# biiiipy/JaxMARL-HFT

Measured on AMD Instinct MI355X. Metric: env steps/sec (whole node), 2-agent MARL, 10-level LOB, NUM_ENVS=4096, higher is better.
Workload: dtype int32

## Files before the change

### jaxmarl-hft_amd/csrc/hftlob.hip

```cpp
#include <hip/hip_runtime.h>
#include <stdint.h>
#include <string.h>
#include <stdio.h>
#include <mutex>
#include <type_traits>
#include <limits.h>

#include "../../include/hftlob.h"
#include "hftlob_internal.h"
#define HFTLOB_BAKED_QUAL static
#include "baked_cfgs.inc"

typedef int32_t i32;
typedef uint32_t u32;
typedef uint8_t u8;
#define DEV __device__ __forceinline__

DEV int lane_id() { return __lane_id(); }
DEV i32 rdl(i32 v, int l) { return __builtin_amdgcn_readlane(v, l); }
DEV i32 wrl(i32 old, i32 val, int l) { return __lane_id() == l ? val : old; }
DEV i32 uni(i32 v) { return __builtin_amdgcn_readfirstlane(v); }
DEV float unif(float v) { return __int_as_float(__builtin_amdgcn_readfirstlane(__float_as_int(v))); }
DEV i32 wadd(i32 a, i32 b) { return (i32)((u32)a + (u32)b); }
DEV i32 wsub(i32 a, i32 b) { return (i32)((u32)a - (u32)b); }
DEV i32 wmul(i32 a, i32 b) { return (i32)((u32)a * (u32)b); }
DEV i32 iabs_(i32 a) { return a < 0 ? wsub(0, a) : a; }
DEV i32 isign(i32 a) { return (a > 0) - (a < 0); }
DEV i32 imax_(i32 a, i32 b) { return a > b ? a : b; }
DEV i32 imin_(i32 a, i32 b) { return a < b ? a : b; }
DEV float i2f(i32 a) { return (float)a; }
DEV i32 f2i(float f) { return (i32)f; }
DEV float bitf(i32 w) { return __int_as_float(w); }
DEV i32 fbit(float f) { return __float_as_int(f); }

DEV i32 ifloordiv(i32 a, i32 b) {
    i32 q = a / b;
    if ((a % b != 0) && ((a < 0) != (b < 0))) q -= 1;
    return q;
}
DEV i32 tick_floordiv(const hftlob_env_cfg& c, i32 a) {
    const u32 d = (u32)c.tick_size;
    const int sh = 31 + (d > 1u ? 32 - __builtin_clz(d - 1u) : 0);
    const u32 n = a < 0 ? ~(u32)a : (u32)a;
    const u32 q = (u32)(((unsigned long long)n * c.tick_magic) >> sh);
    return a < 0 ? (i32)~q : (i32)q;
}
DEV float fmod_exact(float x, float y) {
    const float ax = fabsf(x), ay = fabsf(y), qf = ax / ay;
    if (!(qf < 8388608.0f) | !(ay > 0.0f) | !(ay < INFINITY)) return fmodf(x, y);
    float r = fmaf(-truncf(qf), ay, ax);
    r = r < 0.0f ? r + ay : r;
    return copysignf(r, x);
}
DEV float ffloordiv(float x, float y) {
    float mod = fmod_exact(x, y);
    float div = (x - mod) / y;
    bool ind = (mod != 0.0f) && (((y > 0) - (y < 0)) != ((mod > 0) - (mod < 0)));
    if (ind) div = div - 1.0f;
    return roundf(div);
}

DEV float tick_ffloordiv(const hftlob_env_cfg& c, float x) {
    const float y = (float)c.tick_size, a = fabsf(x);
    const float q = a * __builtin_amdgcn_rcpf(y);
    if (!((a < 16777216.0f) & (q < 524288.0f) & (c.tick_size < (1 << 24)))) return ffloordiv(x, y);
    float k = floorf(q), r = fmaf(-k, y, a);
    if (r < 0.0f) { k -= 1.0f; r += y; }
    else if (r >= y) { k += 1.0f; r -= y; }
    return (x < 0.0f ? -(k + (r != 0.0f ? 1.0f : 0.0f)) : k) + 0.0f;
}

#define DPPX(idv, v, ctrl, rmask) __builtin_amdgcn_update_dpp((idv), (v), (ctrl), (rmask), 0xF, false)
DEV i32 wave_max(i32 v) {
    v = imax_(v, DPPX(INT_MIN, v, 0xB1, 0xF));
    v = imax_(v, DPPX(INT_MIN, v, 0x4E, 0xF));
    v = imax_(v, DPPX(INT_MIN, v, 0x141, 0xF));
    v = imax_(v, DPPX(INT_MIN, v, 0x140, 0xF));
    v = imax_(v, DPPX(INT_MIN, v, 0x142, 0xA));
    v = imax_(v, DPPX(INT_MIN, v, 0x143, 0xC));
    return rdl(v, 63);
}
DEV i32 wave_min(i32 v) {
    v = imin_(v, DPPX(INT_MAX, v, 0xB1, 0xF));
    v = imin_(v, DPPX(INT_MAX, v, 0x4E, 0xF));
    v = imin_(v, DPPX(INT_MAX, v, 0x141, 0xF));
    v = imin_(v, DPPX(INT_MAX, v, 0x140, 0xF));
    v = imin_(v, DPPX(INT_MAX, v, 0x142, 0xA));
    v = imin_(v, DPPX(INT_MAX, v, 0x143, 0xC));
    return rdl(v, 63);
}
DEV i32 wave_sum(i32 v) {
    v = wadd(v, DPPX(0, v, 0xB1, 0xF));
    v = wadd(v, DPPX(0, v, 0x4E, 0xF));
    v = wadd(v, DPPX(0, v, 0x141, 0xF));
    v = wadd(v, DPPX(0, v, 0x140, 0xF));
    v = wadd(v, DPPX(0, v, 0x142, 0xA));
    v = wadd(v, DPPX(0, v, 0x143, 0xC));
    return rdl(v, 63);
}
#define FDPP(v, ctrl, rmask) __int_as_float(DPPX(0, __float_as_int(v), ctrl, rmask))
DEV float wave_fsum(float v) {
    v = v + FDPP(v, 0xB1, 0xF);
    v = v + FDPP(v, 0x4E, 0xF);
    v = v + FDPP(v, 0x141, 0xF);
    v = v + FDPP(v, 0x140, 0xF);
    v = v + FDPP(v, 0x142, 0xA);
    v = v + FDPP(v, 0x143, 0xC);
    return __int_as_float(rdl(__float_as_int(v), 63));
}
DEV unsigned long long ballot(bool p) { return __ballot(p); }
DEV i32 fresh(i32 v) {
    asm volatile("" : "+s"(v));
    return v;
}
DEV i32 sel(bool c, i32 a, i32 b) {
    asm volatile("" : "+v"(a));
    asm volatile("" : "+v"(b));
    return c ? a : b;
}
DEV u32 vkeep(u32 v) {
    asm volatile("" : "+v"(v));
    return v;
}
template <int S> DEV void vkeep_sets(u32 (&v)[S]) {
    if (S == 2) asm volatile("" : "+v"(v[0]), "+v"(v[S - 1]));
    else
#pragma unroll
        for (int r = 0; r < S; ++r) asm volatile("" : "+v"(v[r]));
}
DEV float self(bool c, float a, float b) {
    asm volatile("" : "+v"(a));
    asm volatile("" : "+v"(b));
    return c ? a : b;
}

#ifdef HFTLOB_STAMPS
#define STAMP(var) const unsigned long long var = __builtin_amdgcn_s_memtime()
#ifdef HFTLOB_STAMPS_COARSE
#define SUBSTAMP(var) const unsigned long long var = 0
#define STAMP_ACC(acc, since)
#else
#define SUBSTAMP(var) STAMP(var)
#define STAMP_ACC(acc, since) acc += __builtin_amdgcn_s_memtime() - since
#endif
#else
#define STAMP(var)
#define SUBSTAMP(var)
#define STAMP_ACC(acc, since)
#endif

DEV u32 rotl32(u32 x, int r) { return (x << r) | (x >> (32 - r)); }
DEV void threefry(u32 k0, u32 k1, u32 x0, u32 x1, u32& o0, u32& o1) {
    const u32 k2 = k0 ^ k1 ^ 0x1BD11BDAu;
    x0 += k0;
    x1 += k1;
#define TF_R(r) x0 += x1; x1 = rotl32(x1, r); x1 ^= x0;
#define TF_G1 TF_R(13) TF_R(15) TF_R(26) TF_R(6)
#define TF_G2 TF_R(17) TF_R(29) TF_R(16) TF_R(24)
    TF_G1 x0 += k1; x1 += k2 + 1u;
    TF_G2 x0 += k2; x1 += k0 + 2u;
    TF_G1 x0 += k0; x1 += k1 + 3u;
    TF_G2 x0 += k1; x1 += k2 + 4u;
    TF_G1 x0 += k2; x1 += k0 + 5u;
#undef TF_G1
#undef TF_G2
#undef TF_R
    o0 = x0;
    o1 = x1;
}
struct Key { u32 a, b; };
DEV Key split_key(Key k, int n, int j, bool part) {
    Key o;
    if (part) { threefry(k.a, k.b, 0u, (u32)j, o.a, o.b); return o; }
    u32 y0, y1;
    int m = 2 * j;
    if (m < n) { threefry(k.a, k.b, (u32)m, (u32)(n + m), y0, y1); o.a = y0; }
    else { threefry(k.a, k.b, (u32)(m - n), (u32)m, y0, y1); o.a = y1; }
    m = 2 * j + 1;
    if (m < n) { threefry(k.a, k.b, (u32)m, (u32)(n + m), y0, y1); o.b = y0; }
    else { threefry(k.a, k.b, (u32)(m - n), (u32)m, y0, y1); o.b = y1; }
    return o;
}
DEV u32 random_bits(Key k, int n, int i, bool part) {
    u32 y0, y1;
    if (part) { threefry(k.a, k.b, 0u, (u32)i, y0, y1); return y0 ^ y1; }
    int half = (n + 1) / 2;
    if (i < half) {
        threefry(k.a, k.b, (u32)i, (i + half < n) ? (u32)(i + half) : 0u, y0, y1);
        return y0;
    }
    threefry(k.a, k.b, (u32)(i - half), (i < n) ? (u32)i : 0u, y0, y1);
    return y1;
}
DEV i32 randint_vec(Key k, int n, int j, i32 lo, i32 hi, bool part) {
    Key k1 = split_key(k, 2, 0, part), k2 = split_key(k, 2, 1, part);
    u32 hb = random_bits(k1, n, j, part), lb = random_bits(k2, n, j, part);
    u32 span = (hi <= lo) ? 1u : (u32)hi - (u32)lo;
    u32 mult = 65536u % span;
    mult = (mult * mult) % span;
    u32 off = ((hb % span) * mult + (lb % span)) % span;
    return (i32)((u32)lo + off);
}
DEV i32 action_hi(const hftlob_agent_type_cfg& tc) {
    return tc.kind == HFTLOB_AGENT_EXE && tc.action_space == HFTLOB_EXE_ACT_FIXED_PRICES ? tc.fixed_quant_value
                                                                                         : tc.n_actions;
}
DEV i32 randint(Key k, i32 lo, i32 hi, bool part) { return randint_vec(k, 1, 0, lo, hi, part); }

struct LobCfg {
    i32 maxint, init_id, depth, cancel_mode, t4, check_fill, nO, nT;
};
DEV LobCfg lobcfg(const hftlob_lob_cfg& c) {
    LobCfg o;
    o.maxint = c.maxint; o.init_id = c.init_id; o.depth = c.book_depth; o.cancel_mode = c.cancel_mode;
    o.t4 = c.type_4_interpretation; o.check_fill = c.check_book_fill; o.nO = c.n_orders; o.nT = c.n_trades;
    return o;
}

typedef unsigned long long lmask;
DEV lmask bal(bool p) { return __builtin_amdgcn_ballot_w64(p); }
DEV int ffs64(lmask m) { return m ? (int)__builtin_ctzll(m) : -1; }

extern "C" __device__ i32 __hftlob_writelane(i32 val, i32 lane, i32 old) __asm("llvm.amdgcn.writelane.i32");
DEV i32 wlane(i32 old, i32 val, int l) { return __hftlob_writelane(val, l, old); }

#define ENV_BLOCK 64
DEV void lds_order() { __atomic_signal_fence(__ATOMIC_SEQ_CST); }
DEV void wave_sync() {
    __atomic_signal_fence(__ATOMIC_SEQ_CST);
    __builtin_amdgcn_wave_barrier();
}
DEV void one_wave() {
    if (blockDim.x != ENV_BLOCK) __builtin_trap();
}

enum { FP = 0, FQ, FOID, FTID, FTS, FTNS };

template <int S>
struct Valid {
    lmask m[S];
    bool v[S];
    DEV void init(int n) {
        const int l = lane_id();
#pragma unroll
        for (int r = 0; r < S; ++r) {
            v[r] = (r + 1) * 64 <= n ? true : r * 64 + l < n;
            const int k = n - r * 64;
            m[r] = k >= 64 ? ~0ull : (k <= 0 ? 0ull : ((1ull << k) - 1ull));
        }
    }
};

template <int S> DEV void ldcol(const i32* t, int R, int f, i32 (&o)[S]) {
    const int l = lane_id();
#pragma unroll
    for (int r = 0; r < S; ++r) o[r] = t[f * R + r * 64 + l];
}
DEV i32 ldu(const i32* t, int R, int f, int e) { return uni(t[f * R + e]); }
DEV void ld_msg(const i32* g, int4& x, int4& y) {
    x = reinterpret_cast<const int4*>(g)[0];
    y = reinterpret_cast<const int4*>(g)[1];
}
DEV void stu(i32* t, i32* scr, int R, int f, int e, i32 v) {
    const int l = lane_id();
    *(l == 0 ? t + f * R + e : scr + l) = v;
    lds_order();
}
DEV void st6(i32* t, i32* scr, int R, int e, i32 f0, i32 f1, i32 f2, i32 f3, i32 f4, i32 f5) {
    const int l = lane_id();
    i32 v = f0;
    v = wlane(v, f1, 1); v = wlane(v, f2, 2); v = wlane(v, f3, 3); v = wlane(v, f4, 4); v = wlane(v, f5, 5);
    *(l < 6 ? t + l * R + e : scr + l) = v;
    lds_order();
}
DEV void clr6(i32* t, i32* scr, int R, int e) {
    const int l = lane_id();
    *(l < 6 ? t + l * R + e : scr + l) = -1;
    lds_order();
}
DEV u32 ff1(lmask m) {
    u32 r;
    asm("s_ff1_i32_b64 %0, %1" : "=s"(r) : "s"(m));
    return r;
}
template <int S> DEV int first_slot(const lmask (&m)[S], int fallback) {
    u32 idx = ff1(m[0]);
#pragma unroll
    for (int r = 1; r < S; ++r) idx = min(idx, ff1(m[r]) | (u32)(64 * r));
    return idx == 0xFFFFFFFFu ? fallback : (int)idx;
}
template <int S> DEV int first_true(const bool (&pr)[S], int fallback) {
    lmask m[S];
#pragma unroll
    for (int r = 0; r < S; ++r) m[r] = bal(pr[r]);
    return first_slot(m, fallback);
}
template <int S> DEV i32 sget(const i32 (&a)[S], int e) {
    i32 v = a[0];
#pragma unroll
    for (int k = 1; k < S; ++k) v = (e >> 6) == k ? a[k] : v;
    return rdl(v, e & 63);
}

template <int S>
struct Side {
    i32* t;
    i32* scr;
    i32 best_p, best_q;
    i32 xp;
    i32 pc[S];
    i32 top, top_p, top_ts, top_tns;
    i32 rp, rq;
    lmask rm;
};
template <int S> DEV void side_rec(Side<S>& s, u32 k) {
    s.rp = wlane(s.rp, s.best_p, (int)k);
    s.rq = wlane(s.rq, s.best_q, (int)k);
    asm volatile("s_bitset1_b64 %0, %1" : "+s"(s.rm) : "s"(k));
}

template <int S> DEV void col_set(i32 (&c)[S], int e, i32 v) {
    const int l = lane_id();
#pragma unroll
    for (int r = 0; r < S; ++r) c[r] = (l + 64 * r == e) ? v : c[r];
}

enum : u32 { F_STALE_A = 2, F_STALE_B = 4, F_CLEAN_A = 8, F_CLEAN_B = 16, F_NEG1_A = 32, F_NEG1_B = 64,
             F_PM1_A = 256, F_PM1_B = 512, F_STALE_ANY = 0x40000000u, F_SLOW = 0x80000000u };
constexpr u32 STALE_ANY = F_STALE_ANY;
template <bool ASKS> struct SideBits {
    static constexpr u32 STALE = ASKS ? F_STALE_A : F_STALE_B;
    static constexpr u32 MARK = STALE | STALE_ANY;
    static constexpr u32 CLEAN = ASKS ? F_CLEAN_A : F_CLEAN_B;
    static constexpr u32 NEG1 = ASKS ? F_NEG1_A : F_NEG1_B;
    static constexpr u32 PM1 = ASKS ? F_PM1_A : F_PM1_B;
};
DEV u32 slow_bit(u32 fl) {
    return (fl & (F_CLEAN_A | F_CLEAN_B | F_NEG1_A | F_NEG1_B | F_PM1_A | F_PM1_B)) == (F_CLEAN_A | F_CLEAN_B)
               ? 0u : F_SLOW;
}

template <int S>
struct SideRows {
    int2 x0[S], x1[S], x2[S];
};
template <int S> DEV void fetch_side(SideRows<S>& f, const i32* g, const Valid<S>& V) {
    const int l = lane_id();
#pragma unroll
    for (int r = 0; r < S; ++r) {
        f.x0[r] = f.x1[r] = f.x2[r] = make_int2(-1, -1);
        if (V.v[r]) {
            const int2* row = reinterpret_cast<const int2*>(g + (r * 64 + l) * 6);
            f.x0[r] = row[0]; f.x1[r] = row[1]; f.x2[r] = row[2];
        }
    }
}
template <bool ASKS, int S>
DEV u32 commit_side(Side<S>& s, const SideRows<S>& f, int R, const Valid<S>& V) {
    const int l = lane_id();
    lmask bad = 0, n1 = 0, pm1 = 0;
#pragma unroll
    for (int r = 0; r < S; ++r) {
        const int sl = r * 64 + l;
        const i32 p = f.x0[r].x, q = f.x0[r].y, oid = f.x1[r].x, tid = f.x1[r].y, ts = f.x2[r].x, tns = f.x2[r].y;
        if (V.v[r]) {
            i32* t = s.t + sl;
            t[FP * R] = p; t[FQ * R] = q; t[FOID * R] = oid; t[FTID * R] = tid; t[FTS * R] = ts; t[FTNS * R] = tns;
        }
        s.pc[r] = V.v[r] ? p : -1;
        const u32 np_ = ~(u32)p, nq = ~(u32)q, no = ~(u32)oid, nt = ~(u32)tid, ns = ~(u32)ts, nn = ~(u32)tns;
        const u32 any0 = min(min(min(np_, nq), min(no, nt)), min(ns, nn));
        const u32 all0 = max(max(max(np_, nq), max(no, nt)), max(ns, nn));
        bad |= V.m[r] & bal((q <= 0) & (all0 != 0u));
        n1 |= V.m[r] & bal((p != -1) & (any0 == 0u));
        pm1 |= V.m[r] & bal((p == -1) & (all0 != 0u));
    }
    lds_order();
    s.top = -1;
    return (bad == 0ull ? SideBits<ASKS>::CLEAN : 0u) | (n1 != 0ull ? SideBits<ASKS>::NEG1 : 0u) |
           (pm1 != 0ull ? SideBits<ASKS>::PM1 : 0u);
}
template <int S> DEV void relink_side(Side<S>& s, int R, const Valid<S>& V) {
    i32 p[S];
    ldcol(s.t, R, FP, p);
#pragma unroll
    for (int r = 0; r < S; ++r) s.pc[r] = V.v[r] ? p[r] : -1;
    s.top = -1;
}
template <bool ASKS, int S> DEV u32 load_side(Side<S>& s, const i32* g, int R, const Valid<S>& V) {
    SideRows<S> f;
    fetch_side(f, g, V);
    return commit_side<ASKS>(s, f, R, V);
}
template <int S> DEV void store_side(const Side<S>& s, i32* g, int R, const Valid<S>& V) {
    const int l = lane_id();
#pragma unroll
    for (int r = 0; r < S; ++r) {
        const int sl = r * 64 + l;
        if (V.v[r]) {
            const i32* t = s.t + sl;
            int2* row = reinterpret_cast<int2*>(g + sl * 6);
            row[0] = make_int2(t[FP * R], t[FQ * R]);
            row[1] = make_int2(t[FOID * R], t[FTID * R]);
            row[2] = make_int2(t[FTS * R], t[FTNS * R]);
        }
    }
}
template <int S> DEV void clear_masked(Side<S>& s, int R, const lmask (&m)[S]) {
    const int l = lane_id();
#pragma unroll
    for (int r = 0; r < S; ++r) {
        const bool hit = (m[r] >> l) & 1ull;
        s.pc[r] = hit ? -1 : s.pc[r];
        if (hit) {
#pragma unroll
            for (int f = 0; f < 6; ++f) s.t[f * R + r * 64 + l] = -1;
        }
    }
    lds_order();
    s.top = -1;
}

template <bool ASKS, int S> DEV void rzn(Side<S>& s, u32& fl, int R, const Valid<S>& V) {
    i32 q[S];
    ldcol(s.t, R, FQ, q);
    lmask m[S];
#pragma unroll
    for (int r = 0; r < S; ++r) m[r] = V.m[r] & bal(q[r] <= 0);
    clear_masked(s, R, m);
    fl = fl | SideBits<ASKS>::CLEAN | SideBits<ASKS>::MARK;
    fl = (fl & ~F_SLOW) | slow_bit(fl);
}

template <int S> DEV void best_bid_pq(const i32 (&p)[S], const i32 (&q)[S], const Valid<S>& V, i32& bp, i32& bq) {
    i32 m = INT_MIN;
#pragma unroll
    for (int r = 0; r < S; ++r) m = imax_(m, V.v[r] ? p[r] : INT_MIN);
    const i32 mp = wave_max(m);
    i32 v = 0;
#pragma unroll
    for (int r = 0; r < S; ++r) v = wadd(v, (V.v[r] & (p[r] == mp)) ? q[r] : 0);
    bp = mp;
    bq = wave_sum(v);
}
template <int S>
DEV void best_ask_pq(const i32 (&p)[S], const i32 (&q)[S], const Valid<S>& V, i32 maxint, i32& bp, i32& bq,
                     i32* xp = nullptr) {
    i32 m = INT_MAX;
#pragma unroll
    for (int r = 0; r < S; ++r) m = imin_(m, V.v[r] ? (p[r] == -1 ? maxint : p[r]) : INT_MAX);
    const i32 mn = wave_min(m);
    if (xp) *xp = mn;
    const i32 pa = mn == maxint ? -1 : mn;
    i32 v = 0;
#pragma unroll
    for (int r = 0; r < S; ++r) v = wadd(v, (V.v[r] & (p[r] == pa)) ? q[r] : 0);
    bp = pa;
    bq = wave_sum(v);
}
template <bool ASKS, bool REC, int S>
DEV void rescan(Side<S>& s, u32& fl, int R, const Valid<S>& V, i32 maxint, u32 k) {
    i32 q[S];
    ldcol(s.t, R, FQ, q);
    if (ASKS) best_ask_pq(s.pc, q, V, maxint, s.best_p, s.best_q, &s.xp);
    else best_bid_pq(s.pc, q, V, s.best_p, s.best_q);
    fl &= ~SideBits<ASKS>::STALE;
    if (REC) side_rec(s, k);
}

template <int S>
DEV int top_idx(const i32 (&p)[S], const i32 (&ts)[S], const i32 (&tns)[S], const Valid<S>& V, const LobCfg& c, i32 mp,
                i32& mts_out, i32& mtn_out) {
    i32 t[S], n[S], m = INT_MAX;
#pragma unroll
    for (int r = 0; r < S; ++r) {
        t[r] = (p[r] == mp) ? ts[r] : c.maxint;
        m = imin_(m, V.v[r] ? t[r] : INT_MAX);
    }
    const i32 mts = wave_min(m);
    m = INT_MAX;
#pragma unroll
    for (int r = 0; r < S; ++r) {
        n[r] = (t[r] == mts) ? tns[r] : c.maxint;
        m = imin_(m, V.v[r] ? n[r] : INT_MAX);
    }
    const i32 mtn = wave_min(m);
    mts_out = mts;
    mtn_out = mtn;
    lmask pm[S];
#pragma unroll
    for (int r = 0; r < S; ++r) pm[r] = V.m[r] & bal(n[r] == mtn);
    return first_slot(pm, c.nO - 1);
}

struct Trades {
    i32* t;
    i32* scr;
    int R;
    DEV i32 get(int k, int r) const { return t[k * R + r * 64 + lane_id()]; }
    DEV i32 at(int k, int row) const { return uni(t[k * R + row]); }
};
template <int S> DEV void trades_fill(Trades& T, const Valid<S>& V, i32 v) {
    const int l = lane_id();
#pragma unroll
    for (int r = 0; r < S; ++r)
        if (V.v[r]) {
#pragma unroll
            for (int k = 0; k < 8; ++k) T.t[k * T.R + r * 64 + l] = v;
        }
    lds_order();
}
template <int S> DEV void load_trades(Trades& T, const i32* g, const Valid<S>& V) {
    const int l = lane_id();
#pragma unroll
    for (int r = 0; r < S; ++r) {
        if (V.v[r]) {
            const int o = r * 64 + l, R = T.R;
            const int4* row = reinterpret_cast<const int4*>(g + o * 8);
            const int4 a = row[0], b = row[1];
            T.t[0 * R + o] = a.x; T.t[1 * R + o] = a.y; T.t[2 * R + o] = a.z; T.t[3 * R + o] = a.w;
            T.t[4 * R + o] = b.x; T.t[5 * R + o] = b.y; T.t[6 * R + o] = b.z; T.t[7 * R + o] = b.w;
        }
    }
    lds_order();
}
template <int S> DEV void store_trades(const Trades& T, i32* g, const Valid<S>& V) {
    const int l = lane_id();
#pragma unroll
    for (int r = 0; r < S; ++r) {
        if (V.v[r]) {
            const int o = r * 64 + l, R = T.R;
            int4* row = reinterpret_cast<int4*>(g + o * 8);
            row[0] = make_int4(T.t[0 * R + o], T.t[1 * R + o], T.t[2 * R + o], T.t[3 * R + o]);
            row[1] = make_int4(T.t[4 * R + o], T.t[5 * R + o], T.t[6 * R + o], T.t[7 * R + o]);
        }
    }
}
DEV void trade_put(Trades& T, int e, i32 f0, i32 f1, i32 f2, i32 f3, i32 f4, i32 f5, i32 f6, i32 f7) {
    const int l = lane_id();
    i32 v = f0;
    v = wlane(v, f1, 1); v = wlane(v, f2, 2); v = wlane(v, f3, 3);
    v = wlane(v, f4, 4); v = wlane(v, f5, 5); v = wlane(v, f6, 6); v = wlane(v, f7, 7);
    *(l < 8 ? T.t + l * T.R + e : T.scr + l) = v;
    lds_order();
}

#ifndef HFTLOB_FILT_LOG2
#define HFTLOB_FILT_LOG2 12
#endif
constexpr int FILT_LOG2 = HFTLOB_FILT_LOG2, FILT_WORDS = 1 << (FILT_LOG2 - 5);
constexpr int PAD_FILT = 128, PAD_SCR = PAD_FILT + FILT_WORDS, PAD_WORDS = PAD_SCR + 64;
constexpr int PAD_CARRY = 96;
static_assert(FILT_WORDS >= 64 && FILT_WORDS % 64 == 0 && PAD_WORDS - PAD_SCR == 64, "filter words per lane, 64-word scratch row");
static_assert(PAD_CARRY + 13 <= PAD_FILT, "the rollout's 13 carry words end before the filter words");
__host__ __device__ constexpr int book_words(int nO, int nT) { return 12 * nO + 8 * nT + PAD_WORDS; }
template <int S>
struct Book {
    Side<S> a, b;
    Trades tr;
    Valid<S> vs, vt;
    LobCfg c;
    u32 fl;
    Key ek;
    i32 mi, nmsg;
    i32 ntr;
    bool part;
    i32* filt;
    bool filt_ok;
};

enum { H_ASK = 0, H_BID = 1, H_CNL_ASK = 2, H_CNL_BID = 3, H_NOP = 4, H_KIND = 7, H_DISCARD = 8, H_NEG1 = 16,
       H_PM1 = 32, H_MKT = 64, H_RARE = 128, H_MISS = 256, H_NOID = 512 };
struct Msg {
    i32 h, side, price, qty, oid, tid, t, tns;
    u32 k;
};

template <int S> DEV void top_new(Side<S>& s, int e, i32 np, i32 t, i32 tns, i32 maxint) {
    s.top = ((t != maxint) & (tns != maxint)) ? e : -1;
    s.top_p = np; s.top_ts = t; s.top_tns = tns;
}
template <int S> DEV void top_eq(Side<S>& s, int e, i32 t, i32 tns, i32 maxint) {
    if (fresh(t) > s.top_ts) return;
    asm volatile("");
    if (s.top < 0) return;
    asm volatile("");
    bool earlier = t < s.top_ts;
    if (!earlier) earlier = (tns < s.top_tns) | ((tns == s.top_tns) & (e < s.top));
    if (earlier) {
        s.top = tns != maxint ? e : -1;
        s.top_ts = t; s.top_tns = tns;
    }
}
#define XP_SET(s, v) ((s).xp = (v))
template <bool BID, int S, bool STALE_OK = true, bool NN = false>
DEV void note_add(Side<S>& s, u32& fl, int e, i32 np, i32 nq, i32 t, i32 tns, i32 maxint, u32 k) {
    constexpr u32 STALE = SideBits<!BID>::STALE, MARK = SideBits<!BID>::MARK;
    if (STALE_OK && (fl & STALE)) { s.top = -1; return; }
    const i32 bp = s.best_p;
    if (BID) {
        if (np < bp) {
            if (!NN && bp == -1) fl |= MARK;
        } else if (np > bp) {
            s.best_p = np; s.best_q = nq;
            side_rec(s, k);
            top_new(s, e, np, t, tns, maxint);
        } else if (!NN && bp == -1) {
            fl |= MARK;
        } else {
            s.best_q = wadd(s.best_q, nq);
            side_rec(s, k);
            top_eq(s, e, t, tns, maxint);
        }
    } else if (NN && !STALE_OK) {
        const i32 xp = s.xp;
        if (np > xp) {
        } else if (np < xp) {
            s.best_p = np; s.best_q = nq; XP_SET(s, np); side_rec(s, k); top_new(s, e, np, t, tns, maxint);
        } else if (np == maxint) {
            fl |= MARK;
        } else {
            s.best_q = wadd(s.best_q, nq);
            side_rec(s, k);
            top_eq(s, e, t, tns, maxint);
        }
    } else {
        if (np > bp) {
            if (bp == -1) {
                if (np == maxint) fl |= MARK;
                else { s.best_p = np; s.best_q = nq; XP_SET(s, np); side_rec(s, k); top_new(s, e, np, t, tns, maxint); }
            }
        } else if (np < bp) {
            if (NN || np != -1) { s.best_p = np; s.best_q = nq; XP_SET(s, np); side_rec(s, k); top_new(s, e, np, t, tns, maxint); }
        } else if (!NN && np == -1) {
            fl |= MARK;
        } else if (np != maxint) {
            s.best_q = wadd(s.best_q, nq);
            side_rec(s, k);
            top_eq(s, e, t, tns, maxint);
        }
    }
}
template <bool ASKS, int S> DEV void note_reduce(Side<S>& s, u32& fl, i32 op, i32 dq, u32 k) {
    constexpr u32 STALE = SideBits<ASKS>::STALE, MARK = SideBits<ASKS>::MARK;
    if (fl & STALE) return;
    if (op == s.best_p) {
        if (op == -1) {
            fl |= MARK;
        } else {
            s.best_q = wsub(s.best_q, dq);
            side_rec(s, k);
            if (s.best_q <= 0) fl |= MARK;
        }
    } else {
        asm volatile("");
        u32 f = fl;
        f = fresh(op) == -1 ? f | MARK : f;
        f = fresh(s.best_p) == -1 ? f | MARK : f;
        fl = f;
    }
}

template <int S> DEV void side_put(Side<S>& s, int R, int e, i32 f0, i32 f1, i32 f2, i32 f3, i32 f4, i32 f5) {
    st6(s.t, s.scr, R, e, f0, f1, f2, f3, f4, f5);
    col_set(s.pc, e, f0);
}
template <int S> DEV void side_clr(Side<S>& s, int R, int e) {
    clr6(s.t, s.scr, R, e);
    col_set(s.pc, e, -1);
    s.top = e == s.top ? -1 : s.top;
}
template <int S> DEV void free_slots(const Book<S>& B, const Side<S>& s, lmask (&free)[S]) {
#pragma unroll
    for (int r = 0; r < S; ++r) free[r] = B.vs.m[r] & bal(s.pc[r] == -1);
}

template <int S> DEV bool no_slot(const lmask (&m)[S]) {
    lmask a = 0;
#pragma unroll
    for (int r = 0; r < S; ++r) a |= m[r];
    return a == 0ull;
}

template <bool G, bool ASKS, int S>
DEV i32 match_order(Book<S>& B, Side<S>& s, int top, i32 qtm, const Msg& m, i32 qt, i32 pt, i32 ot, i32 tt) {
    const int R = B.c.nO;
    const i32 newq = imax_(0, wsub(qt, qtm));
    const i32 rem = wsub(qtm, qt);
    int e;
    if (B.ntr >= 0) {
        e = imin_(B.ntr, B.c.nT - 1);
        if (m.t != -1) B.ntr = imin_(B.ntr + 1, B.c.nT);
    } else {
        i32 tr4[S];
        ldcol(B.tr.t, B.tr.R, 4, tr4);
        lmask fm[S];
#pragma unroll
        for (int r = 0; r < S; ++r) fm[r] = B.vt.m[r] & bal(tr4[r] == -1);
        e = first_slot(fm, B.c.nT - 1);
    }
    trade_put(B.tr, e, pt, wmul(wsub(0, m.side), wsub(qt, newq)), ot, m.oid, m.t, m.tns, tt, m.tid);
    if (!G || (B.fl & SideBits<ASKS>::CLEAN)) {
        if (newq <= 0) side_clr(s, R, top);
        else stu(s.t, s.scr, R, FQ, top, newq);
        note_reduce<ASKS>(s, B.fl, pt, wsub(qt, newq), m.k);
    } else {
        stu(s.t, s.scr, R, FQ, top, newq);
        rzn<ASKS>(s, B.fl, R, B.vs);
    }
    return rem;
}

template <bool BID, bool G, int S, bool POS = false>
DEV i32 match_against(Book<S>& B, Side<S>& s, i32 qtm, i32 price, const Msg& m) {
    const int R = B.c.nO;
    if (!POS && fresh(qtm) <= 0) return qtm;
    {
        const i32 bp = s.best_p;
        const i32 mp0 = (!BID && bp == -1) ? B.c.maxint : bp;
        if (__builtin_expect(BID ? mp0 < price : mp0 > price, 1)) return qtm;
    }
    while (qtm > 0) {
        if (B.fl & SideBits<!BID>::STALE) rescan<!BID, true>(s, B.fl, R, B.vs, B.c.maxint, m.k);
        i32 mp = s.best_p;
        if (!BID) {
            if (mp == -1) {
                if (price != B.c.maxint) break;
                mp = B.c.maxint;
            } else if (mp > price) {
                break;
            }
        } else if (mp < price) {
            break;
        }
        int top;
        i32 qt, ot, tt, tp;
        if (s.top >= 0 && s.top_p == mp) {
            top = s.top;
            qt = ldu(s.t, R, FQ, top); ot = ldu(s.t, R, FOID, top); tt = ldu(s.t, R, FTID, top);
            tp = mp;
        } else {
            i32 q[S], o[S], t[S], ts[S], tn[S], mts, mtn;
            ldcol(s.t, R, FTS, ts); ldcol(s.t, R, FTNS, tn);
            ldcol(s.t, R, FQ, q); ldcol(s.t, R, FOID, o); ldcol(s.t, R, FTID, t);
            top = top_idx(s.pc, ts, tn, B.vs, B.c, mp, mts, mtn);
            qt = sget(q, top); ot = sget(o, top); tt = sget(t, top); tp = sget(s.pc, top);
            s.top_p = mp; s.top_ts = mts; s.top_tns = mtn;
            s.top = ((tp == mp) & (mp != -1) & (mp != B.c.maxint) & (mts != B.c.maxint) & (mtn != B.c.maxint))
                        ? top : -1;
        }
        if (fresh(tp) == -1) break;
        asm volatile("");
        if (BID ? tp < price : tp > price) break;
        qtm = match_order<G, !BID>(B, s, top, qtm, m, qt, tp, ot, tt);
    }
    return qtm;
}

template <bool BID, bool G, int S>
DEV void add_order(Book<S>& B, Side<S>& s, const Msg& m, i32 qty, const lmask (&free)[S]) {
    const int R = B.c.nO;
    constexpr u32 CLEAN = SideBits<!BID>::CLEAN, NEG1 = SideBits<!BID>::NEG1, MARK = SideBits<!BID>::MARK,
                  PM1 = SideBits<!BID>::PM1;
    const i32 nq = imax_(0, qty);
    if (!G) {
        const int e = first_slot(free, R - 1);
        const bool was_empty = !no_slot(free);
        if (nq > 0) {
            side_put(s, R, e, m.price, nq, m.oid, m.tid, m.t, m.tns);
            if (m.h & (H_NEG1 | H_PM1)) B.fl = B.fl | (m.h & H_NEG1 ? NEG1 : 0u) | (m.h & H_PM1 ? PM1 : 0u) | F_SLOW;
            if (was_empty) note_add<BID>(s, B.fl, e, m.price, nq, m.t, m.tns, B.c.maxint, m.k);
            else { B.fl |= MARK; s.top = -1; }
        } else if (!was_empty) {
            side_clr(s, R, e);
            B.fl |= MARK;
        }
        return;
    }
    lmask fm[S];
    i32 q[S];
    ldcol(s.t, R, FQ, q);
    if ((B.fl & (CLEAN | NEG1 | PM1)) == CLEAN) {
#pragma unroll
        for (int r = 0; r < S; ++r) fm[r] = free[r];
    } else {
        i32 o[S], t[S], ts[S], tn[S];
        ldcol(s.t, R, FOID, o); ldcol(s.t, R, FTID, t);
        ldcol(s.t, R, FTS, ts); ldcol(s.t, R, FTNS, tn);
#pragma unroll
        for (int r = 0; r < S; ++r)
            fm[r] = B.vs.m[r] & (bal(s.pc[r] == -1) | bal(q[r] == -1) | bal(o[r] == -1) | bal(t[r] == -1) |
                                 bal(ts[r] == -1) | bal(tn[r] == -1));
    }
    const int e = first_slot(fm, R - 1);
    if (!(B.fl & CLEAN)) {
        side_put(s, R, e, m.price, nq, m.oid, m.tid, m.t, m.tns);
        if (m.h & H_PM1) B.fl |= PM1;
        rzn<!BID>(s, B.fl, R, B.vs);
        return;
    }
    const i32 op = sget(s.pc, e), oq = sget(q, e);
    const bool was_empty = (op == -1) & (oq == -1);
    if (nq > 0) {
        side_put(s, R, e, m.price, nq, m.oid, m.tid, m.t, m.tns);
        if (m.h & H_NEG1) B.fl |= NEG1;
        if (m.h & H_PM1) B.fl |= PM1;
        if (was_empty) note_add<BID>(s, B.fl, e, m.price, nq, m.t, m.tns, B.c.maxint, m.k);
        else { B.fl |= MARK; s.top = -1; }
    } else if (!was_empty) {
        side_clr(s, R, e);
        B.fl |= MARK;
    }
}

template <bool BID, int S> DEV void evict_if_full(Book<S>& B, Side<S>& s, lmask (&free)[S]) {
    const int R = B.c.nO;
    lmask neg = 0;
#pragma unroll
    for (int r = 0; r < S; ++r) neg |= B.vs.m[r] & bal(s.pc[r] < 0);
    if (neg != 0ull) return;
    i32 w = BID ? INT_MAX : INT_MIN;
#pragma unroll
    for (int r = 0; r < S; ++r)
        w = BID ? imin_(w, B.vs.v[r] ? s.pc[r] : INT_MAX) : imax_(w, B.vs.v[r] ? s.pc[r] : INT_MIN);
    const i32 worst = BID ? wave_min(w) : wave_max(w);
    lmask m[S];
#pragma unroll
    for (int r = 0; r < S; ++r) m[r] = B.vs.m[r] & bal(s.pc[r] == worst);
    const i32 top = s.top;
    clear_masked(s, R, m);
    s.top = worst != s.top_p ? top : -1;
    if ((worst == s.best_p) | (s.best_p == -1)) B.fl |= SideBits<!BID>::MARK;
#pragma unroll
    for (int r = 0; r < S; ++r) free[r] = m[r];
}
template <bool BID, bool RARE, int S, bool POS = false>
DEV void add_free(Book<S>& B, Side<S>& s, const Msg& m, i32 qty, const lmask (&free)[S]) {
    const int R = B.c.nO;
    if (!POS && qty <= 0) return;
    u32 e;
    if (S == 2) {
        if (free[0] != 0ull) {
            e = ff1(free[0]);
            s.pc[0] = wlane(s.pc[0], m.price, (int)e);
        } else {
            e = ff1(free[S - 1]);
            s.pc[S - 1] = wlane(s.pc[S - 1], m.price, (int)e);
            e |= 64u;
        }
        st6(s.t, s.scr, R, (int)e, m.price, qty, m.oid, m.tid, m.t, m.tns);
    } else {
        e = ff1(free[0]);
#pragma unroll
        for (int r = 1; r < S; ++r) e = min(e, ff1(free[r]) | (u32)(64 * r));
        side_put(s, R, (int)e, m.price, qty, m.oid, m.tid, m.t, m.tns);
    }
    if (RARE && __builtin_expect((m.h & (H_NEG1 | H_PM1)) != 0, 0)) {
        asm volatile("");
        constexpr u32 NEG1 = SideBits<!BID>::NEG1, PM1 = SideBits<!BID>::PM1;
        B.fl = B.fl | (m.h & H_NEG1 ? NEG1 : 0u) | (m.h & H_PM1 ? PM1 : 0u) | F_SLOW;
    }
    note_add<BID, S, false, !RARE>(s, B.fl, (int)e, m.price, qty, m.t, m.tns, B.c.maxint, m.k);
}
template <bool BID, int S> DEV bool add_common(Book<S>& B, Side<S>& s, const Msg& m, const lmask (&free)[S]) {
#ifndef HFTLOB_OLD_ADD_TEST
    if (S == 2) {
        if (__builtin_expect(free[0] != 0ull, 1)) {
            add_free<BID, false, S, true>(B, s, m, m.qty, free);
            return true;
        }
        if (free[S - 1] == 0ull) return false;
        add_free<BID, false, S, true>(B, s, m, m.qty, free);
        return true;
    }
#endif
    if (no_slot(free)) return false;
    add_free<BID, false, S, true>(B, s, m, m.qty, free);
    return true;
}
template <bool G, bool RARE, int S> DEV void bid_lim(Book<S>& B, Msg m) {
    if (!RARE) __builtin_assume(m.qty > 0);
    constexpr bool POS = !RARE && !G;
    if (POS) {
        if (__builtin_expect(B.a.xp > m.price, 1)) {
            lmask free[S];
            free_slots(B, B.b, free);
            if (add_common<true>(B, B.b, m, free)) return;
            if (B.c.check_fill) evict_if_full<true>(B, B.b, free);
            add_order<true, G>(B, B.b, m, m.qty, free);
            return;
        }
    }
    const i32 rem = match_against<false, G, S, POS>(B, B.a, m.qty, m.price, m);
    if (RARE && __builtin_expect((m.h & H_MKT) != 0, 0)) m.price = B.c.maxint;
    lmask free[S];
    free_slots(B, B.b, free);
    if (!no_slot(free)) {
        if (!G) add_free<true, RARE>(B, B.b, m, (RARE && (m.h & H_DISCARD)) ? 0 : rem, free);
        else if (!(m.h & H_DISCARD)) add_order<true, G>(B, B.b, m, rem, free);
        return;
    }
    if (B.c.check_fill) evict_if_full<true>(B, B.b, free);
    if (!(m.h & H_DISCARD)) add_order<true, G>(B, B.b, m, rem, free);
}
template <bool G, bool RARE, int S> DEV void ask_lim(Book<S>& B, Msg m) {
    if (!RARE) __builtin_assume(m.qty > 0);
    if (RARE && __builtin_expect((m.h & H_MKT) != 0, 0)) m.price = 0;
    constexpr bool POS = !RARE && !G;
    if (POS && __builtin_expect(B.b.best_p < m.price, 1)) {
        lmask free[S];
        free_slots(B, B.a, free);
        if (add_common<false>(B, B.a, m, free)) return;
        if (B.c.check_fill) evict_if_full<false>(B, B.a, free);
        add_order<false, G>(B, B.a, m, m.qty, free);
        return;
    }
    const i32 rem = match_against<true, G, S, POS>(B, B.b, m.qty, m.price, m);
    lmask free[S];
    free_slots(B, B.a, free);
    if (!no_slot(free)) {
        if (!G) add_free<false, RARE>(B, B.a, m, (RARE && (m.h & H_DISCARD)) ? 0 : rem, free);
        else if (!(m.h & H_DISCARD)) add_order<false, G>(B, B.a, m, rem, free);
        return;
    }
    if (B.c.check_fill) evict_if_full<false>(B, B.a, free);
    if (!(m.h & H_DISCARD)) add_order<false, G>(B, B.a, m, rem, free);
}
template <int S>
DEV int random_id_match(const Book<S>& B, Key& k, const i32 (&o)[S], const lmask (&pm)[S]) {
    k = split_key(k, 2, 0, B.part);
    lmask w[S];
    int tot = 0;
#pragma unroll
    for (int r = 0; r < S; ++r) {
        w[r] = pm[r] & bal(o[r] != 0);
        tot += __builtin_popcountll(w[r]);
    }
    const u32 bits = random_bits(k, 1, 0, B.part);
    const float u = __uint_as_float((bits >> 9) | 0x3f800000u) - 1.0f;
    const float rr = (float)tot * (1.0f - u);
    i32 chosen = 0;
    if (tot > 0) {
        int K = (int)ceilf(rr);
#pragma unroll
        for (int r = 0; r < S; ++r) {
            const int c = __builtin_popcountll(w[r]);
            if (K > 0 && K <= c) {
                const u32 below = __builtin_amdgcn_mbcnt_hi((u32)(w[r] >> 32), __builtin_amdgcn_mbcnt_lo((u32)w[r], 0u));
                const lmask hit = w[r] & bal(below == (u32)(K - 1));
                chosen = rdl(o[r], (int)ff1(hit));
            }
            K -= c;
        }
    }
    lmask f[S];
#pragma unroll
    for (int r = 0; r < S; ++r) f[r] = B.vs.m[r] & bal(o[r] == chosen);
    return first_slot(f, -1);
}
template <bool G, bool ASKS, bool RC, int S> DEV void cancel(Book<S>& B, Side<S>& s, const Msg& m) {
    if (!G && m.qty == 0) return;
    const int R = B.c.nO;
    int idx;
    i32 op, oq;
    if (!RC && (m.h & H_MISS)) {
        idx = R - 1;
        op = sget(s.pc, R - 1);
#ifndef HFTLOB_NO_MISS_EMPTY
        if (!G && fresh(op) == -1) return;
        asm volatile("");
#endif
        oq = ldu(s.t, R, FQ, R - 1);
    } else {
    i32 o[S], q[S];
    ldcol(s.t, R, FOID, o);
    ldcol(s.t, R, FQ, q);
    lmask fm[S];
    idx = -1;
    if (RC || !(m.h & H_NOID)) {
#pragma unroll
        for (int r = 0; r < S; ++r) fm[r] = B.vs.m[r] & bal(o[r] == m.oid);
        idx = first_slot(fm, -1);
    }
    if (idx < 0) {
        const i32 lo = wsub(B.c.init_id, wmul(B.c.depth, 2));
        const u32 span = (u32)wsub(B.c.init_id, lo);
        u32 d[S];
#pragma unroll
        for (int r = 0; r < S; ++r) d[r] = (u32)wsub(o[r], lo);
        vkeep_sets(d);
#pragma unroll
        for (int r = 0; r < S; ++r) d[r] = s.pc[r] == m.price ? d[r] : 0xFFFFFFFFu;
        vkeep_sets(d);
#pragma unroll
        for (int r = 0; r < S; ++r) d[r] = q[r] >= m.qty ? d[r] : 0xFFFFFFFFu;
        vkeep_sets(d);
#pragma unroll
        for (int r = 0; r < S; ++r) fm[r] = B.vs.m[r] & bal(d[r] <= span);
        if (!RC) {
            idx = first_slot(fm, R - 1);
        } else {
            idx = first_slot(fm, -1);
            if (idx < 0 && B.c.cancel_mode >= 2) {
                Key k = split_key(B.ek, B.nmsg, B.mi, B.part);
#pragma unroll
                for (int r = 0; r < S; ++r) fm[r] = B.vs.m[r] & bal(s.pc[r] == m.price) & bal(q[r] >= m.qty);
                idx = random_id_match(B, k, o, fm);
                if (idx < 0 && B.c.cancel_mode == 3) {
#pragma unroll
                    for (int r = 0; r < S; ++r) fm[r] = B.vs.m[r] & bal(s.pc[r] == m.price);
                    idx = random_id_match(B, k, o, fm);
                }
            }
            if (idx < 0) idx = R - 1;
        }
    }
    op = sget(s.pc, idx);
    oq = sget(q, idx);
    }
    if (!G && fresh(op & oq) == -1) {
        asm volatile("");
        if (m.qty >= -1) return;
#ifndef HFTLOB_NO_MISS_EMPTY
        B.fl |= SideBits<ASKS>::PM1 | F_SLOW;
#endif
    }
    const i32 nq = wsub(oq, m.qty);
    if (!G || (B.fl & SideBits<ASKS>::CLEAN)) {
        if (nq <= 0) side_clr(s, R, idx);
        else stu(s.t, s.scr, R, FQ, idx, nq);
        note_reduce<ASKS>(s, B.fl, op, wsub(oq, nq > 0 ? nq : 0), m.k);
    } else {
        stu(s.t, s.scr, R, FQ, idx, nq);
        rzn<ASKS>(s, B.fl, R, B.vs);
    }
}

DEV void decode_msgs(const LobCfg& c, int4& x, const int4& y) {
    const i32 ty = x.x, sd = ty == 4 ? wsub(0, x.y) : x.y;
    const bool cnl = (ty == 2) | (ty == 3);
    i32 h = H_ASK;
    h = (((ty == 0) & (sd == 0))) ? H_NOP : h;
    h = (((ty == 1) | (ty == 4)) & (sd == 1)) ? H_BID : h;
    h = (cnl & (sd == 1)) ? H_CNL_BID : h;
    h = (cnl & (sd == -1)) ? H_CNL_ASK : h;
    if (((c.t4 == 0) | (c.t4 == 2)) & (ty == 4)) h |= H_DISCARD;
    const i32 p_add = c.t4 == 2 ? (h == H_BID ? c.maxint : 0) : x.w;
    if ((p_add != -1) & ((y.x == -1) | (y.y == -1) | (y.z == -1) | (y.w == -1))) h |= H_NEG1;
    if (p_add == -1) h |= H_PM1;
    if (c.t4 == 2) h |= H_MKT;
    if (h & (H_DISCARD | H_NEG1 | H_PM1 | H_MKT)) h |= H_RARE;
    if ((h <= H_BID) & (x.z <= 0)) h |= H_RARE;
    if (((h & H_KIND) == H_ASK) & (sd != -1)) h |= H_RARE;
    if ((h <= H_BID) & (x.w < 0)) h |= H_RARE;
    x.x = h;
    x.y = sd;
}
template <bool G, bool RC, int S>
DEV void process_msg_(Book<S>& B, u32 k, i32 h, i32 sdv, i32 d2, i32 d3, i32 d4, i32 d5, i32 d6, i32 d7) {
    Msg m;
    m.h = h; m.side = 0; m.price = d3; m.qty = d2; m.oid = d4; m.tid = d5; m.t = d6; m.tns = d7;
    m.k = k;
    const i32 kind = h & H_KIND;
    if (kind == H_CNL_ASK) cancel<G, true, RC>(B, B.a, m);
    else if (kind == H_CNL_BID) cancel<G, false, RC>(B, B.b, m);
    else if (kind == H_BID) {
        if (!G && !(h & H_RARE)) {
            m.side = 1;
            bid_lim<G, false>(B, m);
        } else {
            m.side = rdl(sdv, k);
            bid_lim<G, true>(B, m);
        }
    } else if (kind == H_ASK) {
        if (!G && !(h & H_RARE)) {
            m.side = -1;
            ask_lim<G, false>(B, m);
        } else {
            m.side = rdl(sdv, k);
            ask_lim<G, true>(B, m);
        }
    }
}

DEV i32 ffill(i32 v, i32 carry) {
    const int l = lane_id();
    const lmask m = bal(v != -1) & (~0ull >> (63 - l));
    const int src = m ? 63 - __builtin_clzll(m) : -1;
    const i32 got = __builtin_amdgcn_ds_bpermute(src << 2, v);
    return src < 0 ? carry : got;
}
template <bool REC = true, int S> DEV void refresh_best(Book<S>& B, u32 k = 0) {
    if (B.fl & STALE_ANY) {
        if (B.fl & F_STALE_A) rescan<true, REC>(B.a, B.fl, B.c.nO, B.vs, B.c.maxint, k);
        if (B.fl & F_STALE_B) rescan<false, REC>(B.b, B.fl, B.c.nO, B.vs, B.c.maxint, k);
        B.fl &= ~STALE_ANY;
    }
}

DEV u32 hash_id(i32 v) { return ((u32)v * 0x9E3779B1u) >> (32 - FILT_LOG2); }
DEV u32 hash_px(i32 p, bool ask) { return (((u32)p * 0x85EBCA6Bu) ^ (ask ? 0xC2B2AE35u : 0x27D4EB2Fu)) >> (32 - FILT_LOG2); }
DEV void filt_set(i32* f, u32 h, bool on) {
    __hip_atomic_fetch_or(reinterpret_cast<u32*>(f) + (h >> 5), on ? 1u << (h & 31) : 0u, __ATOMIC_RELAXED,
                          __HIP_MEMORY_SCOPE_WORKGROUP);
}
DEV u32 filt_get(const i32* f, u32 h) { return ((u32)f[h >> 5] >> (h & 31)) & 1u; }
DEV u32 lanes_below(lmask m) { return __builtin_amdgcn_mbcnt_hi((u32)(m >> 32), __builtin_amdgcn_mbcnt_lo((u32)m, 0u)); }
template <int S> DEV int side_room(const Book<S>& B, const Side<S>& s) {
    const int R = B.c.nO, rl = (R - 1) >> 6, ll = (R - 1) & 63;
    int n = 0;
    bool last = false;
#pragma unroll
    for (int r = 0; r < S; ++r) {
        lmask f = B.vs.m[r] & bal(s.pc[r] == -1);
        if (r == rl) {
            last = (f >> ll) & 1ull;
            f &= ~(1ull << ll);
        }
        n += __builtin_popcountll(f);
    }
    if (!last) return -1;
    return ldu(s.t, R, FQ, R - 1) == -1 ? n : -1;
}
template <bool RC, int S> DEV lmask chunk_noops(Book<S>& B, const int4& x, const int4& y, int cnt, i32& hf) {
    const int l = lane_id();
    const i32 kind = x.x & H_KIND, qty = x.z, price = x.w, oid = y.x;
    const bool in = l < cnt;
    const lmask nop = bal(in & (kind == H_NOP));
    hf = 0;
    if ((i32)B.fl < 0) {
        B.filt_ok = false;
        return nop;
    }
    const bool cnl = (kind == H_CNL_ASK) | (kind == H_CNL_BID), add = (kind == H_ASK) | (kind == H_BID);
    const i32 lo = wsub(B.c.init_id, wmul(B.c.depth, 2));
    const u32 span = (u32)wsub(B.c.init_id, lo);
    const bool init_oid = (u32)wsub(oid, lo) <= span;
    const lmask brk = bal(in & ((add & (((x.x & (H_NEG1 | H_PM1)) != 0) | init_oid)) | (cnl & (qty < -1))));
    const lmask before = brk ? (1ull << ff1(brk)) - 1ull : ~0ull;
    const lmask zero = bal(in & cnl & (qty == 0)) & before;
    if (RC || (u32)wsub(-1, lo) <= span) return nop | zero;
    i32* f = B.filt;
    if (!B.filt_ok) {
#pragma unroll
        for (int w = 0; w < FILT_WORDS; w += 64) f[w + l] = 0;
        wave_sync();
        const int R = B.c.nO;
#pragma unroll
        for (int sd = 0; sd < 2; ++sd) {
            const Side<S>& s = sd ? B.b : B.a;
            i32 o[S];
            ldcol(s.t, R, FOID, o);
#pragma unroll
            for (int r = 0; r < S; ++r) {
                filt_set(f, hash_id(o[r]), B.vs.v[r] & (o[r] != -1));
                filt_set(f, hash_px(s.pc[r], sd == 0), B.vs.v[r] & ((u32)wsub(o[r], lo) <= span));
            }
        }
    }
    filt_set(f, hash_id(oid), in & add);
    B.filt_ok = brk == 0ull;
    wave_sync();
    const bool ask = kind == H_CNL_ASK;
    const u32 hid = filt_get(f, hash_id(oid)), hpx = filt_get(f, hash_px(price, ask));
    const bool hit = (hid | hpx) != 0u;
    const int room_a = side_room(B, B.a), room_b = side_room(B, B.b);
    const u32 adds_a = lanes_below(bal(in & (kind == H_ASK))), adds_b = lanes_below(bal(in & (kind == H_BID)));
    const int room = ask ? room_a : room_b;
    const i32 adds = (i32)(ask ? adds_a : adds_b);
    const bool cmiss = in & cnl & (oid != -1) & !hit;
    const bool quiet = cmiss & (qty >= -1) & (room >= 0) & (adds <= room);
#ifndef HFTLOB_NO_MISS
    const bool cnd = in & cnl & (oid != -1) & (hid == 0u) & (((before >> l) & 1ull) != 0ull);
    hf = cnd ? (hpx == 0u ? (i32)H_MISS : (i32)H_NOID) : 0;
#endif
    return nop | zero | (bal(quiet) & before);
}

#ifdef HFTLOB_STAMPS_CHUNK
#define CHUNK_PARAMS , unsigned long long &acc_pre, unsigned long long &acc_loop
#define CHUNK_ARGS , acc_pre, acc_loop
#else
#define CHUNK_PARAMS
#define CHUNK_ARGS
#endif
template <bool RC, int S>
DEV void run_chunk(Book<S>& B, const int4& x, const int4& y, int cnt, int base, i32& rpa, i32& rqa, i32& rpb,
                   i32& rqb CHUNK_PARAMS) {
#ifdef HFTLOB_STAMPS_CHUNK
    const unsigned long long tp0 = __builtin_amdgcn_s_memtime();
#endif
    const lmask live = cnt >= 64 ? ~0ull : (1ull << cnt) - 1ull;
#ifdef HFTLOB_NO_SKIP
    const lmask skip = 0;
    const i32 hx = x.x;
#else
    i32 hf;
    const lmask skip = chunk_noops<RC>(B, x, y, cnt, hf) & live;
    const i32 hx = x.x | hf;
#endif
    lmask todo = live & ~skip;
#ifdef HFTLOB_KO_LOOP
    todo = 0;
#endif
    refresh_best<false>(B);
    const i32 cpa = B.a.best_p, cqa = B.a.best_q, cpb = B.b.best_p, cqb = B.b.best_q;
    B.a.rm = B.b.rm = 0ull;
    B.a.rp = B.a.rq = B.b.rp = B.b.rq = 0;
#ifdef HFTLOB_STAMPS_CHUNK
    const unsigned long long tp1 = __builtin_amdgcn_s_memtime();
    acc_pre += tp1 - tp0;
#endif
    if (todo) {
        u32 k = ff1(todo);
        i32 h = rdl(hx, k), d2 = rdl(x.z, k), d3 = rdl(x.w, k), d4 = rdl(y.x, k),
            d5 = rdl(y.y, k), d6 = rdl(y.z, k), d7 = rdl(y.w, k);
        do {
            asm volatile("s_bitset0_b64 %0, %1" : "+s"(todo) : "s"(k));
            if (RC) B.mi = base + (int)k;
            if ((i32)B.fl >= 0) process_msg_<false, RC>(B, k, h, x.y, d2, d3, d4, d5, d6, d7);
            else process_msg_<true, RC>(B, k, h, x.y, d2, d3, d4, d5, d6, d7);
            refresh_best(B, k);
            const u32 kn = ff1(todo);
            h = rdl(hx, kn); d2 = rdl(x.z, kn); d3 = rdl(x.w, kn);
            d4 = rdl(y.x, kn); d5 = rdl(y.y, kn); d6 = rdl(y.z, kn); d7 = rdl(y.w, kn);
            k = kn;
        } while (todo);
    }
#ifdef HFTLOB_STAMPS_CHUNK
    acc_loop += __builtin_amdgcn_s_memtime() - tp1;
#endif
    {
        const int l = lane_id();
        const lmask below = ~0ull >> (63 - l);
        const lmask ma = B.a.rm & below, mb = B.b.rm & below;
        const int sa = ma ? 63 - __builtin_clzll(ma) : -1, sb = mb ? 63 - __builtin_clzll(mb) : -1;
        const i32 gpa = __builtin_amdgcn_ds_bpermute(sa << 2, B.a.rp), gqa = __builtin_amdgcn_ds_bpermute(sa << 2, B.a.rq);
        const i32 gpb = __builtin_amdgcn_ds_bpermute(sb << 2, B.b.rp), gqb = __builtin_amdgcn_ds_bpermute(sb << 2, B.b.rq);
        rpa = sa < 0 ? cpa : gpa;
        rqa = sa < 0 ? cqa : gqa;
        rpb = sb < 0 ? cpb : gpb;
        rqb = sb < 0 ? cqb : gqb;
    }
}

template <int S> DEV void book_bind(Book<S>& B, i32* lds) {
    B.a.t = lds;
    B.b.t = lds + 6 * B.c.nO;
    B.tr.t = lds + 12 * B.c.nO;
    B.tr.R = B.c.nT;
    B.filt = lds + 12 * B.c.nO + 8 * B.c.nT + PAD_FILT;
    B.filt_ok = false;
    B.a.scr = B.b.scr = B.tr.scr = lds + 12 * B.c.nO + 8 * B.c.nT + PAD_SCR;
    B.vs.init(B.c.nO);
    B.vt.init(B.c.nT);
}

template <int S, bool RC>
__global__ __launch_bounds__(64) void k_book_process(hftlob_lob_cfg cfg, int n_env, int n_msg, const u32* __restrict__ keys,
                                                     const i32* __restrict__ msgs,
                                                     i32* __restrict__ asks, i32* __restrict__ bids,
                                                     i32* __restrict__ trades, i32* __restrict__ best_asks,
                                                     i32* __restrict__ best_bids) {
    one_wave();
    extern __shared__ __attribute__((aligned(16))) i32 lds[];
    const int e = blockIdx.x;
    if (e >= n_env) return;
    const int l = lane_id();
    Book<S> B;
    B.c = lobcfg(cfg);
    book_bind(B, lds);
    const int R = B.c.nO;
    i32* ga = asks + (size_t)e * R * 6;
    i32* gb = bids + (size_t)e * R * 6;
    i32* gt = trades + (size_t)e * B.c.nT * 8;
    B.fl = load_side<true>(B.a, ga, R, B.vs) | load_side<false>(B.b, gb, R, B.vs) | F_STALE_A | F_STALE_B | STALE_ANY;
    B.fl |= slow_bit(B.fl);
    load_trades(B.tr, gt, B.vt);
    {
        lmask fr[S], bad = 0;
#pragma unroll
        for (int r = 0; r < S; ++r) fr[r] = B.vt.m[r] & bal(B.tr.get(4, r) == -1);
        const int first = first_slot(fr, B.c.nT);
        const int l = lane_id();
#pragma unroll
        for (int r = 0; r < S; ++r) bad |= B.vt.m[r] & ~fr[r] & bal(r * 64 + l >= first);
        B.ntr = bad == 0ull ? first : -1;
    }
    if (RC) {
        B.ek = Key{keys[2 * e], keys[2 * e + 1]};
        B.nmsg = n_msg;
        B.part = cfg.prng_partitionable;
    }
    const i32* gm = msgs + (size_t)e * n_msg * 8;
    int4 nx = make_int4(0, 0, 0, 0), ny = nx;
    if (l < n_msg) {
        ld_msg(gm + l * 8, nx, ny);
    }
    for (int base = 0; base < n_msg; base += 64) {
        const int row = base + l;
        int4 x = nx, y = ny;
        nx = make_int4(0, 0, 0, 0);
        ny = nx;
        if (row + 64 < n_msg) {
            ld_msg(gm + (row + 64) * 8, nx, ny);
        }
        decode_msgs(B.c, x, y);
        i32 ap = 0, aq = 0, bp = 0, bq = 0;
        const int cnt = uni(imin_(64, n_msg - base));
#ifdef HFTLOB_STAMPS_CHUNK
        unsigned long long acc_pre = 0, acc_loop = 0;
#endif
        run_chunk<RC>(B, x, y, cnt, base, ap, aq, bp, bq CHUNK_ARGS);
        if (best_asks && row < n_msg) {
            reinterpret_cast<int2*>(best_asks + ((size_t)e * n_msg + row) * 2)[0] = make_int2(ap, aq);
            reinterpret_cast<int2*>(best_bids + ((size_t)e * n_msg + row) * 2)[0] = make_int2(bp, bq);
        }
    }
    store_side(B.a, ga, R, B.vs);
    store_side(B.b, gb, R, B.vs);
    store_trades(B.tr, gt, B.vt);
}

struct EnvCfg {
    const hftlob_env_cfg* c;
};

enum { LD_T0 = 0, LD_T1, LD_WIN, LD_MAXS, LD_START, LD_STEP };
enum { W_T0 = 0, W_T1, W_OIDC, W_MID, W_DT };

DEV int agent_words(const hftlob_agent_type_cfg& t) { return t.kind == HFTLOB_AGENT_MM ? 5 : 13; }

template <int S> DEV i32 side_volume_pq(const i32 (&p)[S], const i32 (&q)[S], const Valid<S>& V) {
    i32 v = 0;
#pragma unroll
    for (int r = 0; r < S; ++r) v = wadd(v, (V.v[r] && p[r] != -1) ? q[r] : 0);
    return wave_sum(v);
}
template <int S> DEV i32 side_volume(const Side<S>& s, int R, const Valid<S>& V) {
    i32 q[S];
    ldcol(s.t, R, FQ, q);
    return side_volume_pq(s.pc, q, V);
}
template <int S> DEV void global_pq(const i32* g, const Valid<S>& V, i32 (&p)[S], i32 (&q)[S]) {
    const int l = lane_id();
#pragma unroll
    for (int r = 0; r < S; ++r) {
        p[r] = q[r] = -1;
        if (V.v[r]) {
            const int2 x = reinterpret_cast<const int2*>(g + (r * 64 + l) * 6)[0];
            p[r] = x.x; q[r] = x.y;
        }
    }
}

struct DivBatch {
    int l;
    float n = 0.0f, d = 1.0f, q = 0.0f;
    DEV void add(int k, float num, float den) {
        n = l == k ? num : n;
        d = l == k ? den : d;
    }
    DEV void run() { q = n / d; }
    DEV float get(int k) const { return unif_lane(q, k); }
    DEV static float unif_lane(float v, int k) { return __int_as_float(__builtin_amdgcn_readlane(__float_as_int(v), k)); }
};
DEV float zsum(float z, int n) { return n >= 64 ? z : z + 0.0f; }
template <int S> DEV float rows_fsum(const float (&x)[S], int n) {
    const int l = lane_id();
    float a = l < n ? x[0] : 0.0f;
#pragma unroll
    for (int r = 1; r < S; ++r) if (r * 64 + l < n) a = a + x[r];
    return wave_fsum(a);
}

struct ObsLane {
    int l;
    float v = 0.0f, off = 0.0f, div = 1.0f;
    DEV void put(int k, float x, float o, float d) {
        const bool me = l == k;
        v = me ? x : v;
        off = me ? o : off;
        div = me ? d : div;
    }
    DEV void put_i(int k, i32 x) { v = l == k ? __int_as_float(x) : v; }
    DEV float fin() const { return (v - off) / div; }
};

struct WorldView {
    i32 best_ask_p, best_bid_p, vol_a, vol_b, step, max_steps;
    float mid;
    i32 t0, t1, it0, it1;
    float dt;
};

#define OBS_F(k, x, o_, d_) o.put((k), (x), nz ? (o_) : 0.0f, nz ? (d_) : 1.0f)
#define OBS_I(k, x, o_, d_) do { if (RAW) o.put_i((k), (x)); else OBS_F((k), i2f(x), (o_), (d_)); } while (0)
template <bool RAW>
DEV void mm_obs(const hftlob_env_cfg& c, const hftlob_agent_type_cfg& tc, const WorldView& w, const i32* st, ObsLane& o,
                bool ftime) {
    const bool nz = !RAW && tc.normalize;
    const i32 spread = iabs_(wsub(w.best_ask_p, w.best_bid_p));
    if (tc.observation_space == HFTLOB_MM_OBS_BASIC) {
        OBS_I(0, st[2], 0.0f, 10.0f);
        OBS_I(1, spread, 0.0f, 1e4f);
        return;
    }
    if (tc.observation_space == HFTLOB_MM_OBS_MESSAGES) return;
    if (ftime) {
        const float tm = i2f(w.t0) + i2f(w.t1) / 1e9f;
        const float trem = (float)c.episode_time - (tm - (i2f(w.it0) + i2f(w.it1) / 1e9f));
        OBS_F(0, w.dt, 0.0f, 10.0f);
        OBS_I(1, st[2], 0.0f, 10.0f);
        OBS_F(2, w.mid, 0.0f, 1e6f);
        OBS_I(3, w.best_ask_p, 0.0f, 1e6f);
        OBS_I(4, w.best_bid_p, 0.0f, 1e6f);
        OBS_I(5, w.vol_a, 0.0f, 1000.0f);
        OBS_I(6, w.vol_b, 0.0f, 1000.0f);
        OBS_I(7, spread, 0.0f, 1e4f);
        OBS_I(8, w.step, 0.0f, 10.0f);
        OBS_F(9, trem, 0.0f, (float)c.episode_time);
        return;
    }
    OBS_I(0, st[2], 0.0f, 10.0f);
    OBS_F(1, w.mid, 0.0f, 1e6f);
    OBS_I(2, w.best_ask_p, 0.0f, 1e6f);
    OBS_I(3, w.best_bid_p, 0.0f, 1e6f);
    OBS_I(4, w.vol_a, 0.0f, 1000.0f);
    OBS_I(5, w.vol_b, 0.0f, 1000.0f);
    OBS_I(6, spread, 0.0f, 1e4f);
    OBS_I(7, w.step, 0.0f, 10.0f);
}
template <bool RAW>
DEV void exe_obs(const hftlob_env_cfg& c, const hftlob_agent_type_cfg& tc, const WorldView& w, const i32* st, ObsLane& o,
                 bool ftime) {
    const bool nz = !RAW && tc.normalize;
    if (tc.observation_space == HFTLOB_EXE_OBS_BASIC) {
        const i32 rq = wsub(st[1], st[2]);
        if (RAW) {
            o.put_i(0, w.best_ask_p);
            o.put_i(1, w.best_bid_p);
        } else {
            o.put(0, i2f(nz ? wsub(w.best_ask_p, 1550000) : w.best_ask_p), 0.0f, nz ? 1e3f : 1.0f);
            o.put(1, i2f(nz ? wsub(w.best_bid_p, 1550000) : w.best_bid_p), 0.0f, nz ? 1e3f : 1.0f);
        }
        OBS_I(2, rq, 0.0f, (float)tc.task_size);
        return;
    }
    if (tc.observation_space == HFTLOB_EXE_OBS_SIMPLEST_CASE) {
        const float ep = (float)c.episode_time;
        const float ptr = (ep - (i2f(wsub(w.t0, w.it0)) + i2f(wsub(w.t1, w.it1)) / 1e9f)) / ep;
        const float prq = i2f(wsub(st[1], st[2])) / i2f(st[1]);
        OBS_F(0, w.mid, 7560000.0f, 1e3f);
        OBS_F(1, prq, 0.5f, 1.0f);
        OBS_F(2, ptr, 0.5f, 1.0f);
        return;
    }
    const i32 sell = st[3];
    const i32 p_aggr = sell ? w.best_bid_p : w.best_ask_p, p_pass = sell ? w.best_ask_p : w.best_bid_p;
    const i32 q_aggr = sell ? w.vol_b : w.vol_a, q_pass = sell ? w.vol_a : w.vol_b;
    const float ip = bitf(st[0]);
    const float ts = (float)tc.task_size;
    const float rr = w.max_steps == 0 ? 0.0f : 1.0f - i2f(w.step) / i2f(w.max_steps);
    const i32 spr = iabs_(wsub(p_aggr, p_pass)), rq = wsub(st[1], st[2]);
    int k = 0;
    if (ftime) {
        OBS_F(0, w.dt, 0.0f, 10.0f);
        k = 1;
    }
    OBS_I(k + 0, st[2], 0.0f, ts);
    OBS_F(k + 1, ip, 0.0f, 1e7f);
    OBS_I(k + 2, sell, 0.0f, 1.0f);
    OBS_I(k + 3, p_aggr, ip, 1e5f);
    OBS_I(k + 4, p_pass, ip, 1e5f);
    OBS_I(k + 5, q_aggr, 0.0f, 1000.0f);
    OBS_I(k + 6, q_pass, 0.0f, 1000.0f);
    OBS_I(k + 7, rq, 0.0f, ts);
    OBS_F(k + 8, rr, 0.0f, 1.0f);
    OBS_I(k + 9, spr, 0.0f, 1e4f);
    OBS_I(k + 10, w.step, 0.0f, 30.0f);
    OBS_I(k + 11, st[1], 0.0f, ts);
    if (ftime) {
        const float tm = i2f(w.t0) + i2f(w.t1) / 1e9f;
        const float trem = (float)c.episode_time - (tm - (i2f(w.it0) + i2f(w.it1) / 1e9f));
        OBS_F(13, tm, 0.0f, 1e5f);
        OBS_F(14, trem, 0.0f, (float)c.episode_time);
    }
}
#undef OBS_I
#undef OBS_F
template <bool RAW>
DEV void write_obs(const hftlob_env_cfg& c, const hftlob_agent_type_cfg& tc, const WorldView& w, const i32* st,
                   void* dst, bool zero, bool ftime) {
    const int l = lane_id();
    ObsLane o{l};
    if (tc.kind == HFTLOB_AGENT_MM) mm_obs<RAW>(c, tc, w, st, o, ftime);
    else exe_obs<RAW>(c, tc, w, st, o, ftime);
    const float v = zero ? 0.0f : (RAW ? o.v : o.fin());
    if (l < c.obs_stride) static_cast<float*>(dst)[l] = v;
}

static_assert(HFTLOB_N_BAKED == 4, "baked_cfg names the table's entries one by one");
template <int BAKED> DEV const hftlob_env_cfg& baked_cfg(const hftlob_env_cfg& rt) {
    static_assert(BAKED >= -1 && BAKED < HFTLOB_N_BAKED, "no such baked config");
    if constexpr (BAKED == 0) return hftlob_baked_cfg_0;
    else if constexpr (BAKED == 1) return hftlob_baked_cfg_1;
    else if constexpr (BAKED == 2) return hftlob_baked_cfg_2;
    else if constexpr (BAKED == 3) return hftlob_baked_cfg_3;
    else return rt;
}
template <int BAKED> constexpr int baked_unroll() { return BAKED >= 0 ? HFTLOB_MAX_AGENTS : 1; }

template <int S, int BAKED = -1>
DEV void env_reset_dev(const hftlob_env_cfg& c_rt, Key key, const i32* __restrict__ init_states, i32* __restrict__ rec,
                       float* __restrict__ obs, const Valid<S>& VS, const Valid<S>& VT, bool ftime) {
    const hftlob_env_cfg& c = baked_cfg<BAKED>(c_rt);
    constexpr int UNR = baked_unroll<BAKED>();
    const bool part = c.prng_partitionable;
    const int nTy = c.n_types, l = lane_id();
    Key wk = split_key(key, nTy + 1, nTy, part);
    i32 idx = c.window_selector == -1 ? randint(wk, 0, c_rt.n_windows, part) : c.window_selector;
    idx = imin_(imax_(idx, 0), c_rt.n_windows - 1);
    const i32* src = init_states + (size_t)idx * c.init_rec_words;
    for (int w = l * 4; w < c.init_rec_words; w += 256) {
        if (w + 3 < c.init_rec_words) {
            *reinterpret_cast<int4*>(rec + w) = *reinterpret_cast<const int4*>(src + w);
        } else {
            for (int k = w; k < c.init_rec_words; ++k) rec[k] = src[k];
        }
    }
    i32 ap[S], aq[S], bp[S], bq[S], ba_p, ba_q, bb_p, bb_q;
    global_pq(src + c.off_asks, VS, ap, aq);
    global_pq(src + c.off_bids, VS, bp, bq);
    best_ask_pq(ap, aq, VS, c.lob.maxint, ba_p, ba_q);
    best_bid_pq(bp, bq, VS, bb_p, bb_q);
    for (int m = l; m < c.n_msgs; m += 64) {
        reinterpret_cast<int2*>(rec + c.off_best_asks)[m] = make_int2(ba_p, ba_q);
        reinterpret_cast<int2*>(rec + c.off_best_bids)[m] = make_int2(bb_p, bb_q);
    }
    const float mid = i2f(wadd(bb_p, ba_p)) / 2.0f;
    const i32 t0 = src[c.off_loaded + LD_T0], t1 = src[c.off_loaded + LD_T1];
    if (l == 0) {
        i32* W = rec + c.off_world;
        W[W_T0] = t0; W[W_T1] = t1; W[W_OIDC] = c.order_id_counter_start; W[W_MID] = fbit(mid); W[W_DT] = fbit(0.0f);
    }
    WorldView wv;
    wv.best_ask_p = ba_p; wv.best_bid_p = bb_p;
    wv.vol_a = side_volume_pq(ap, aq, VS); wv.vol_b = side_volume_pq(bp, bq, VS);
    wv.step = src[c.off_loaded + LD_STEP]; wv.max_steps = src[c.off_loaded + LD_MAXS]; wv.mid = mid;
    wv.t0 = wv.it0 = t0; wv.t1 = wv.it1 = t1; wv.dt = 0.0f;
    int agents_end = c.off_agents;
#pragma unroll UNR
    for (int t = 0; t < nTy; ++t) agents_end += c.types[t].n_agents * agent_words(c.types[t]);
    for (int w = c.off_world + 5 + l; w < c.off_agents; w += 64) rec[w] = 0;
    for (int w = agents_end + l; w < c.rec_words; w += 64) rec[w] = 0;
    i32* st = rec + c.off_agents;
    int ag = 0;
#pragma unroll UNR
    for (int t = 0; t < nTy; ++t) {
        const hftlob_agent_type_cfg& tc = c.types[t];
        i32 sell = tc.task == HFTLOB_TASK_SELL ? 1 : 0;
        if (tc.kind == HFTLOB_AGENT_EXE && tc.task == HFTLOB_TASK_RANDOM)
            sell = randint(split_key(key, nTy + 1, t, part), 0, 2, part);
#pragma unroll UNR
        for (int i = 0; i < tc.n_agents; ++i, ++ag) {
            i32 s[13];
            if (tc.kind == HFTLOB_AGENT_MM) {
                s[0] = 0; s[1] = 0; s[2] = 0; s[3] = fbit(0.0f); s[4] = fbit(0.0f);
            } else {
                s[0] = fbit(mid); s[1] = tc.task_size; s[2] = 0; s[3] = sell; s[4] = fbit(mid / (float)c.tick_size);
                for (int k = 5; k < 13; ++k) s[k] = fbit(0.0f);
            }
            const int nw = agent_words(tc);
            i32 v = 0;
            for (int k = 0; k < 13; ++k) if (l == k) v = s[k];
            if (l < nw) st[l] = v;
            if (obs) write_obs<false>(c, tc, wv, s, obs + (size_t)ag * c.obs_stride, false, ftime);
            st += nw;
        }
    }
}

template <int S>
__global__ __launch_bounds__(64) void k_env_reset(hftlob_env_cfg c, int n_env, const u32* __restrict__ keys,
                                                  const i32* __restrict__ init_states, i32* __restrict__ state,
                                                  float* __restrict__ obs) {
    one_wave();
    const int e = blockIdx.x;
    if (e >= n_env) return;
    Valid<S> VS, VT;
    VS.init(c.lob.n_orders);
    VT.init(c.lob.n_trades);
    Key k{keys[2 * e], keys[2 * e + 1]};
    env_reset_dev<S>(c, k, init_states, state + (size_t)e * c.rec_words,
                     obs ? obs + (size_t)e * c.n_agents * c.obs_stride : nullptr, VS, VT, c.ep_type == 1);
}

struct ActX {
    i32 bid_price, ask_price, bid_dist, ask_dist, bid_quant, ask_quant;
};

DEV void put_row(i32* lds_rows, int row, i32 f0, i32 f1, i32 f2, i32 f3, i32 f4, i32 f5, i32 f6, i32 f7) {
    const int l = lane_id();
    i32 v = f0;
    v = l == 1 ? f1 : v; v = l == 2 ? f2 : v; v = l == 3 ? f3 : v;
    v = l == 4 ? f4 : v; v = l == 5 ? f5 : v; v = l == 6 ? f6 : v; v = l == 7 ? f7 : v;
    if (l < 8) lds_rows[row * 8 + l] = v;
}

template <int S>
struct RegRows {
    int4 x, y;
    i32 meta;
    i32 at[S], aq[S], ao[S], bt[S], bq[S], bo[S];
    DEV void init(const i32* ta, const i32* tb, int R, int C, i32 t, i32 tns) {
        const int l = lane_id();
        const bool cl = l < C;
        x = make_int4(cl ? 2 : 0, 0, 0, 0);
        y = make_int4(0, 0, cl ? t : 0, cl ? tns : 0);
        meta = l | l << 8;
        ldcol(ta, R, FTID, at); ldcol(ta, R, FQ, aq); ldcol(ta, R, FOID, ao);
        ldcol(tb, R, FTID, bt); ldcol(tb, R, FQ, bq); ldcol(tb, R, FOID, bo);
    }
    DEV void put(int row, i32 f0, i32 f1, i32 f2, i32 f3, i32, i32, i32, i32) {
        const bool m = lane_id() == row;
        x.x = m ? f0 : x.x; x.y = m ? f1 : x.y; x.z = m ? f2 : x.z; x.w = m ? f3 : x.w;
    }
    DEV void agent(int arow, int crow, int n, i32 tid, i32 t, i32 tns) {
        const int l = lane_id();
        const bool ia = (u32)(l - arow) < (u32)n, ic = (u32)(l - crow) < (u32)n;
        y.y = ia ? tid : y.y; y.z = ia ? t : y.z; y.w = ia ? tns : y.w;
        const i32 ma = arow | crow << 8 | (n - 1) << 16, mc = crow | arow << 8 | (n - 1) << 16;
        meta = ia ? ma : (ic ? mc : meta);
    }
};
template <int S>
DEV void put_row(RegRows<S>* r, int row, i32 f0, i32 f1, i32 f2, i32 f3, i32 f4, i32 f5, i32 f6, i32 f7) {
    r->put(row, f0, f1, f2, f3, f4, f5, f6, f7);
}
template <class T> struct is_reg_rows { static constexpr bool value = false; };
template <int S> struct is_reg_rows<RegRows<S>*> { static constexpr bool value = true; };
template <bool REG, int S> DEV auto row_sink(RegRows<S>& regs, i32* lds_rows) {
    if constexpr (REG) return &regs;
    else return lds_rows;
}
template <int S>
DEV void cancel_regs(RegRows<S>& sink, const i32 (&tid)[S], const i32 (&q)[S], const i32 (&o)[S], const i32 (&p)[S],
                     const Valid<S>& V, i32 agent, int size, i32 side, int row0) {
    const int l = lane_id();
    sink.x.y = (u32)(l - row0) < (u32)size ? side : sink.x.y;
    int n = 0;
#pragma unroll
    for (int r = 0; r < S; ++r) {
        lmask bm = V.m[r] & bal(tid[r] == agent);
        while (bm && n < size) {
            const int ln = (int)__builtin_ctzll(bm);
            bm &= bm - 1;
            const bool m = l == row0 + n;
            sink.x.z = m ? rdl(q[r], ln) : sink.x.z; sink.x.w = m ? rdl(p[r], ln) : sink.x.w;
            sink.y.x = m ? rdl(o[r], ln) : sink.y.x; sink.y.y = m ? agent : sink.y.y;
            ++n;
        }
    }
}

template <int S>
DEV void cancel_rows(const Side<S>& s, int R, const Valid<S>& V, i32 agent, int size, i32 side, i32 t, i32 tns,
                     i32* lds_rows, int row0) {
    int n = 0;
    i32 tid[S], q[S], o[S];
    const i32 (&p)[S] = s.pc;
    ldcol(s.t, R, FTID, tid);
    ldcol(s.t, R, FQ, q);
    ldcol(s.t, R, FOID, o);
#pragma unroll
    for (int r = 0; r < S; ++r) {
        lmask bm = V.m[r] & bal(tid[r] == agent);
        while (bm && n < size) {
            const int ln = (int)__builtin_ctzll(bm);
            bm &= bm - 1;
            put_row(lds_rows, row0 + n, 2, side, rdl(q[r], ln), rdl(p[r], ln), rdl(o[r], ln), agent, t, tns);
            ++n;
        }
    }
    for (; n < size; ++n) put_row(lds_rows, row0 + n, 2, side, 0, 0, 0, 0, t, tns);
}

template <int n>
DEV void filter_rows(i32* lds_rows, int arow, int crow, i32* scratch) {
    wave_sync();
    const int l = lane_id();
    const bool is_a = l < n, is_c = (l >= 8) & (l < 8 + n);
    const int row = is_a ? arow + l : (is_c ? crow + l - 8 : arow);
    const i32 p = lds_rows[row * 8 + 3], q = lds_rows[row * 8 + 2];
    lmask ma = 0, mc = 0;
#pragma unroll
    for (int k = 0; k < n; ++k) {
        const i32 cpk = rdl(p, 8 + k), apk = rdl(p, k);
        ma |= bal(is_a & (p != 0) & (p == cpk));
        mc |= bal(is_c & (apk != 0) & (p == apk));
    }
    constexpr lmask amask = (1ull << n) - 1, cmask = amask << 8;
    const int na = __builtin_popcountll(ma), nc = __builtin_popcountll(mc);
    const lmask mine = is_a ? ma : mc, all = is_a ? amask : cmask;
    const bool matched = (mine >> l) & 1ull;
    const lmask below = matched ? mine : (~mine & all);
    const int cnt = (int)__builtin_amdgcn_mbcnt_hi((u32)(below >> 32), __builtin_amdgcn_mbcnt_lo((u32)below, 0u));
    const int rank = matched ? cnt : (is_a ? na : nc) + cnt;
    if (l < 16) scratch[l] = 0;
    wave_sync();
    if ((is_a | is_c) & matched) scratch[(is_c ? 8 : 0) + rank] = q;
    wave_sync();
    const i32 av = scratch[rank & 7], cv = scratch[8 + (rank & 7)];
    const i32 nq = wsub(q, cv >= av ? av : 0);
    if (is_a & (nq == 0)) {
        reinterpret_cast<int4*>(lds_rows + row * 8)[0] = make_int4(0, 0, 0, 0);
        reinterpret_cast<int4*>(lds_rows + row * 8)[1] = make_int4(0, 0, 0, 0);
    } else if (is_a | is_c) {
        lds_rows[row * 8 + 2] = nq;
    }
    wave_sync();
}
template <int S>
DEV void filter_regs(RegRows<S>& s, int C) {
    const int l = lane_id();
    const int own = s.meta & 0xFF, oth = (s.meta >> 8) & 0xFF, g1 = s.meta >> 16, off = l - own;
    const i32 p = s.x.w, q = s.x.z;
    bool hit = false;
#pragma unroll
    for (int r = 0; r < 4; ++r) hit |= __builtin_amdgcn_ds_bpermute((oth + ((off + r) & g1)) << 2, p) == p;
    const bool matched = hit & (p != 0);
    const lmask M = bal(matched);
    const u32 grp = (u32)(M >> own) & ((2u << g1) - 1u);
    const int mb = __builtin_popcount(grp & ((1u << off) - 1u));
    const int rank = matched ? mb : __builtin_popcount(grp) + off - mb;
    const bool is_a = l >= C;
    const int slot = ((is_a ? own : oth) + rank) << 2;
    const i32 av = __builtin_amdgcn_ds_permute((matched & is_a) ? slot : 0, q);
    const i32 cv = __builtin_amdgcn_ds_permute((matched & !is_a) ? slot : 0, q);
    const i32 nq = wsub(q, __builtin_amdgcn_ds_bpermute(slot, cv >= av ? av : 0));
    if (is_a & (nq == 0)) {
        s.x = make_int4(0, 0, 0, 0);
        s.y = s.x;
    } else {
        s.x.z = nq;
    }
}

template <int S, class Rows>
DEV bool masked_best(const hftlob_env_cfg& c, Book<S>& B, const Rows lds_rows, i32 tid, i32 last_ba, i32 last_bb, i32& ba,
                     i32& bb) {
    const i32 tick = c.tick_size;
    i32 mn = INT_MAX, mx = INT_MIN, at_[S], bt_[S];
    const i32 (&ap_)[S] = B.a.pc;
    const i32 (&bp_)[S] = B.b.pc;
    if constexpr (is_reg_rows<Rows>::value) {
#pragma unroll
        for (int r = 0; r < S; ++r) { at_[r] = lds_rows->at[r]; bt_[r] = lds_rows->bt[r]; }
    } else {
        ldcol(B.a.t, B.c.nO, FTID, at_);
        ldcol(B.b.t, B.c.nO, FTID, bt_);
    }
#pragma unroll
    for (int r = 0; r < S; ++r) {
        const i32 pa = (B.vs.v[r] && at_[r] != tid) ? ap_[r] : -1;
        const i32 pb = (B.vs.v[r] && bt_[r] != tid) ? bp_[r] : -1;
        mn = imin_(mn, B.vs.v[r] ? (pa == -1 ? c.lob.maxint : pa) : INT_MAX);
        mx = imax_(mx, B.vs.v[r] ? pb : INT_MIN);
    }
    ba = wave_min(mn);
    bb = wave_max(mx);
    ba = ba == c.lob.maxint ? -1 : ba;
    const bool empty = (ba == -1) || (bb == -1);
    ba = wmul(tick_floordiv(c, ba), tick);
    bb = wmul(tick_floordiv(c, bb), tick);
    if (empty) { bb = last_bb; ba = last_ba; }
    return empty;
}
template <int S, class Rows>
DEV void mm_fixed_quant(const hftlob_env_cfg& c, const hftlob_agent_type_cfg& tc, Book<S>& B, const i32* st, i32 tid,
                        i32 action, i32 wt0, i32 wt1, i32 last_ba, i32 last_bb, Rows lds_rows, int row, ActX& x) {
    if (tc.fixed_action_setting) action = tc.fixed_action;
    const i32 tick = c.tick_size;
    i32 ba, bb;
    const bool empty = masked_best(c, B, lds_rows, tid, last_ba, last_bb, ba, bb);
    const float hsp = fmaxf(i2f(wsub(ba, bb)) / 2.0f, (float)tick / 2.0f);
    const float hs = (tick_ffloordiv(c, hsp) + 1.0f) * (float)tick;
    float bo, ao;
    i32 bq, aq;
    if (!tc.sell_buy_all_option) {
        const int ai = action < 0 ? imax_(action + 10, 0) : (action > 9 ? 9 : action);
        bo = (float)((0x0152043210ull >> (4 * ai)) & 0xF);
        ao = (float)((0x0510243210ull >> (4 * ai)) & 0xF);
        const i32 q1 = ai == 9 ? 0 : 1;
        bq = wmul(q1, tc.fixed_quant_value);
        aq = wmul(q1, tc.fixed_quant_value);
    } else {
        const int ai = action < 0 ? imax_(action + 9, 0) : (action > 8 ? 8 : action);
        const i32 bot[9] = {10, 2, 4, -1, 0, 2, -20, 0, 0}, aot[9] = {10, 2, 4, -1, 2, 0, 0, -20, 0};
        const i32 iq = ifloordiv(st[2], tc.fixed_quant_value);
        i32 b = bot[0], a = aot[0];
#pragma unroll
        for (int k = 1; k < 9; ++k) { b = ai == k ? bot[k] : b; a = ai == k ? aot[k] : a; }
        bo = i2f(b);
        ao = i2f(a);
        bq = wmul(ai < 6 ? 1 : (ai == 6 ? iq : 0), tc.fixed_quant_value);
        aq = wmul(ai < 6 ? 1 : (ai == 7 ? iq : 0), tc.fixed_quant_value);
    }
    if (empty) { bq = 0; aq = 0; }
    const float bpf = i2f(bb) - bo * hs;
    const float apf = i2f(ba) + ao * hs;
    const i32 bp = f2i(tick_ffloordiv(c, fmaxf(bpf, 0.0f)) * (float)tick);
    const i32 ap = f2i(tick_ffloordiv(c, fmaxf(i2f(wadd(bp, tick)), apf)) * (float)tick);
    i32 typ0 = 1, typ1 = 1, sd0 = 1, sd1 = -1, qq0 = bq, qq1 = aq, pp0 = bp, pp1 = ap;
// ... 695 lines not shown
    const Key key{(u32)__builtin_amdgcn_ds_bpermute(b0 << 2, ka), (u32)__builtin_amdgcn_ds_bpermute(b0 << 2, kb2)};
    const bool hi_lane = ll >= 12;
    const int ag = ll - (hi_lane ? 12 : 8);
    int t = 0, i = 0;
    agent_of_lane(c, ag < 0 ? 0 : ag, t, i);
    const bool agent_lane = (ll >= 8) & (ag >= 0) & (ag < c.n_agents);
    const Key L1 = split_key(key, ll < 2 ? 2 : nTy, ll < 2 ? ll : ll - 2, part);
    const Key P2 = from_lane(L1, b0 + (agent_lane ? 2 + t : 0));
    const Key L2 = split_key(P2, agent_lane ? type_n_agents(c, t) : 2, agent_lane ? i : 1, part);
    const Key L3 = split_key(L2, 2, ((ll == 0) | hi_lane) ? 1 : 0, part);
    const Key sub = from_lane(L3, b0);
    const u32 bits = random_bits(ll < A ? sub : L3, 1, ll < A ? ll : 0, part);
    const u32 hb = bits, lb = (u32)__builtin_amdgcn_ds_bpermute(((l + 4) & 63) << 2, (i32)bits);
    const i32 na = agent_lane ? type_action_hi(c, t, MD) : 1;
    const u32 span = na <= 0 ? 1u : (u32)na;
    u32 mult = 65536u % span;
    mult = (mult * mult) % span;
    const i32 act = (i32)(((hb % span) * mult + (lb % span)) % span);
    const i32 l1a = __builtin_amdgcn_ds_bpermute((b0 + ((ll >> 2) & 1)) << 2, (i32)L1.a);
    const i32 l1b = __builtin_amdgcn_ds_bpermute((b0 + ((ll >> 2) & 1)) << 2, (i32)L1.b);
    const i32 ac = __builtin_amdgcn_ds_bpermute((b0 + 8 + (ll >= 6 ? ll - 6 : 0)) << 2, act);
    const i32 sh = __builtin_amdgcn_ds_bpermute((b0 + (ll >= 6 + c.n_agents ? ll - 6 - c.n_agents : 0)) << 2, (i32)bits);
    i32 w = ll == 0 ? (i32)key.a : (ll == 1 ? (i32)key.b : ((ll & 1) ? l1b : l1a));
    w = ll >= 6 + c.n_agents ? sh : (ll >= 6 ? ac : w);
    if ((j < nb) & (ll < KW)) kb[j * KW + ll] = w;
    wave_sync();
}
DEV StepKeys load_keys(const hftlob_env_cfg& c, const i32* row) {
    const int l = lane_id(), na = c.n_agents, A = c.n_action_msgs;
    StepKeys o;
    o.key = Key{(u32)uni(row[0]), (u32)uni(row[1])};
    o.k1 = Key{(u32)uni(row[2]), (u32)uni(row[3])};
    o.key_reset = Key{(u32)uni(row[4]), (u32)uni(row[5])};
    o.next_master = Key{0u, 0u};
    const int ag = l - 32;
    o.acts = ((ag >= 0) & (ag < na)) ? row[6 + (ag < 0 ? 0 : ag)] : 0;
    o.shuffle_bits = l < A ? (u32)row[6 + na + (l < A ? l : 0)] : 0u;
    return o;
}

DEV void fixed_time_mask(int4& x, int4& y, i32 t_end) {
    if (y.z >= t_end) {
        x = make_int4(0, 0, 0, 0);
        y.x = 0;
        y.y = 0;
    }
}

template <bool BID, int S>
DEV i32 l2_side(const Side<S>& s, int R, const Valid<S>& V, i32 maxint, i32 outv) {
    const int l = lane_id();
    i32 x[S], q[S];
    ldcol(s.t, R, FQ, q);
#pragma unroll
    for (int r = 0; r < S; ++r) x[r] = BID ? wmul(-1, s.pc[r]) : (s.pc[r] == -1 ? maxint : s.pc[r]);
    i32 prev = 0;
    for (int k = 0; k < HFTLOB_L2_LEVELS; ++k) {
        i32 m = INT_MAX;
        lmask any = 0;
#pragma unroll
        for (int r = 0; r < S; ++r) {
            const bool ok = V.v[r] && (k == 0 || x[r] > prev);
            m = imin_(m, ok ? x[r] : INT_MAX);
            any |= bal(ok);
        }
        i32 lv = wave_min(m);
        if (any == 0ull) lv = BID ? 1 : -1;
        else prev = lv;
        i32 p = BID ? wmul(-1, lv) : lv;
        p = p == -1 ? (BID ? wsub(0, maxint) : maxint) : p;
        i32 v = 0;
#pragma unroll
        for (int r = 0; r < S; ++r) v = wadd(v, (V.v[r] && s.pc[r] == p) ? q[r] : 0);
        const i32 vol = imax_(wave_sum(v), 0);
        const int c = k * 4 + (BID ? 2 : 0);
        outv = l == c ? p : (l == c + 1 ? vol : outv);
    }
    return outv;
}
template <int S> DEV void write_debug(const Book<S>& B, i32* dst) {
    const int l = lane_id(), R = B.c.nO;
    i32 v = 0;
    v = l2_side<false>(B.a, R, B.vs, B.c.maxint, v);
    v = l2_side<true>(B.b, R, B.vs, B.c.maxint, v);
    if (l < 4 * HFTLOB_L2_LEVELS) dst[l] = v;
    store_trades(B.tr, dst + 4 * HFTLOB_L2_LEVELS, B.vt);
}

template <bool BID, int S>
DEV i32 depth_side(const Side<S>& s, int R, const Valid<S>& V, i32 maxint, int n_levels, i32 outv) {
    const int l = lane_id();
    i32 x[S], q[S];
    ldcol(s.t, R, FQ, q);
#pragma unroll
    for (int r = 0; r < S; ++r) x[r] = BID ? wmul(-1, s.pc[r]) : (s.pc[r] == -1 ? maxint : s.pc[r]);
    i32 prev = 0;
    for (int k = 0; k < n_levels; ++k) {
        i32 m = INT_MAX;
        lmask any = 0;
#pragma unroll
        for (int r = 0; r < S; ++r) {
            const bool ok = V.v[r] && (k == 0 || x[r] > prev);
            m = imin_(m, ok ? x[r] : INT_MAX);
            any |= bal(ok);
        }
        i32 lv = wave_min(m);
        if (any == 0ull) lv = BID ? 1 : -1;
        else prev = lv;
        i32 p = BID ? wmul(-1, lv) : lv;
        p = p == -1 ? (BID ? wsub(0, maxint) : maxint) : p;
        i32 v = 0;
#pragma unroll
        for (int r = 0; r < S; ++r) v = wadd(v, (V.v[r] && s.pc[r] == p) ? q[r] : 0);
        const i32 vol = imax_(wave_sum(v), 0);
        const int c = k * 4 + (BID ? 2 : 0);
        outv = l == c ? p : (l == c + 1 ? vol : outv);
    }
    return outv;
}

template <int S>
__global__ __launch_bounds__(64) void k_book_depth(hftlob_lob_cfg cfg, int n_env, int n_levels,
                                                   const i32* __restrict__ asks, const i32* __restrict__ bids,
                                                   i32* __restrict__ depth) {
    one_wave();
    extern __shared__ __attribute__((aligned(16))) i32 lds[];
    const int e = blockIdx.x;
    if (e >= n_env) return;
    const int l = lane_id();
    Book<S> B;
    B.c = lobcfg(cfg);
    book_bind(B, lds);
    const int R = B.c.nO;
    load_side<true>(B.a, asks + (size_t)e * R * 6, R, B.vs);
    load_side<false>(B.b, bids + (size_t)e * R * 6, R, B.vs);
    i32 v = 0;
    v = depth_side<false>(B.a, R, B.vs, B.c.maxint, n_levels, v);
    v = depth_side<true>(B.b, R, B.vs, B.c.maxint, n_levels, v);
    if (l < 4 * n_levels) depth[(size_t)e * 4 * n_levels + l] = v;
}

template <int S, bool RC>
__global__ __launch_bounds__(64) void k_book_process_depth(hftlob_lob_cfg cfg, int n_env, int n_msg,
                                                           const u32* __restrict__ keys, const i32* __restrict__ msgs,
                                                           i32* __restrict__ asks, i32* __restrict__ bids,
                                                           i32* __restrict__ trades, int n_levels, int n_keep,
                                                           i32* __restrict__ depth, i32* __restrict__ all_asks,
                                                           i32* __restrict__ all_bids) {
    one_wave();
    extern __shared__ __attribute__((aligned(16))) i32 lds[];
    const int e = blockIdx.x;
    if (e >= n_env) return;
    const int l = lane_id();
    Book<S> B;
    B.c = lobcfg(cfg);
    book_bind(B, lds);
    const int R = B.c.nO;
    i32* ga = asks + (size_t)e * R * 6;
    i32* gb = bids + (size_t)e * R * 6;
    i32* gt = trades + (size_t)e * B.c.nT * 8;
    B.fl = load_side<true>(B.a, ga, R, B.vs) | load_side<false>(B.b, gb, R, B.vs) | F_STALE_A | F_STALE_B | STALE_ANY;
    B.fl |= slow_bit(B.fl);
    load_trades(B.tr, gt, B.vt);
    {
        lmask fr[S], bad = 0;
#pragma unroll
        for (int r = 0; r < S; ++r) fr[r] = B.vt.m[r] & bal(B.tr.get(4, r) == -1);
        const int first = first_slot(fr, B.c.nT);
#pragma unroll
        for (int r = 0; r < S; ++r) bad |= B.vt.m[r] & ~fr[r] & bal(r * 64 + l >= first);
        B.ntr = bad == 0ull ? first : -1;
    }
    if (RC) {
        B.ek = Key{keys[2 * e], keys[2 * e + 1]};
        B.nmsg = n_msg;
        B.part = cfg.prng_partitionable;
    }
    const int first_kept = n_msg - n_keep;
    const int dw = 4 * n_levels;
    i32* gd = depth ? depth + (size_t)e * n_keep * dw : nullptr;
    i32* gsa = all_asks ? all_asks + (size_t)e * n_keep * R * 6 : nullptr;
    i32* gsb = all_asks ? all_bids + (size_t)e * n_keep * R * 6 : nullptr;
    i32 dv = 0;
    u32 dirty = 3u;
    const i32* gm = msgs + (size_t)e * n_msg * 8;
    int4 nx = make_int4(0, 0, 0, 0), ny = nx;
    if (l < n_msg) {
        ld_msg(gm + l * 8, nx, ny);
    }
    for (int base = 0; base < n_msg; base += 64) {
        const int row = base + l;
        int4 x = nx, y = ny;
        nx = make_int4(0, 0, 0, 0);
        ny = nx;
        if (row + 64 < n_msg) {
            ld_msg(gm + (row + 64) * 8, nx, ny);
        }
        decode_msgs(B.c, x, y);
        const int cnt = uni(imin_(64, n_msg - base));
        const lmask live = cnt >= 64 ? ~0ull : (1ull << cnt) - 1ull;
        i32 hf;
        const lmask skip = chunk_noops<RC>(B, x, y, cnt, hf) & live;
        const i32 hx = x.x | hf;
        refresh_best<false>(B);
        B.a.rm = B.b.rm = 0ull;
        B.a.rp = B.a.rq = B.b.rp = B.b.rq = 0;
        for (int k = 0; k < cnt; ++k) {
            if (!((skip >> k) & 1ull)) {
                const i32 h = rdl(hx, k), d2 = rdl(x.z, k), d3 = rdl(x.w, k), d4 = rdl(y.x, k), d5 = rdl(y.y, k),
                          d6 = rdl(y.z, k), d7 = rdl(y.w, k);
                const i32 ntr0 = B.ntr;
                if (RC) B.mi = base + k;
                if ((i32)B.fl >= 0) process_msg_<false, RC>(B, (u32)k, h, x.y, d2, d3, d4, d5, d6, d7);
                else process_msg_<true, RC>(B, (u32)k, h, x.y, d2, d3, d4, d5, d6, d7);
                refresh_best(B, (u32)k);
#ifdef HFTLOB_DEPTH_BOTH
                (void)ntr0;
                dirty = 3u;
#else
                const i32 kind = h & H_KIND;
                const bool add = kind <= H_BID;
                const bool no_trade = (ntr0 >= 0) & (ntr0 < B.c.nT) & (B.ntr == ntr0) & (d6 != -1);
                dirty |= ((kind == H_ASK) | (kind == H_CNL_ASK)) ? 1u : 2u;
                if (add & !no_trade) dirty = 3u;
#endif
            }
            const int j = base + k - first_kept;
            if (j >= 0) {
                if (gd) {
                    if (dirty & 1u) dv = depth_side<false>(B.a, R, B.vs, B.c.maxint, n_levels, dv);
                    if (dirty & 2u) dv = depth_side<true>(B.b, R, B.vs, B.c.maxint, n_levels, dv);
                    dirty = 0u;
                    if (l < dw) gd[(size_t)j * dw + l] = dv;
                }
                if (gsa) {
                    store_side(B.a, gsa + (size_t)j * R * 6, R, B.vs);
                    store_side(B.b, gsb + (size_t)j * R * 6, R, B.vs);
                }
            }
        }
    }
    store_side(B.a, ga, R, B.vs);
    store_side(B.b, gb, R, B.vs);
    store_trades(B.tr, gt, B.vt);
}

#define MAX_AGENT_ROWS 128

constexpr u32 INFO_F32_MM = 0xC0B9FFu, INFO_F32_EXE = 0x13Cu;
constexpr u32 TALLY_SUM_LANES = 0x34u;
struct TallyLane { double a, b; };
DEV int tally_word(int l) { return l < 25 ? 8 + 2 * l : (l < 40 ? l - 32 : 58 + 2 * (l - 40)); }
DEV TallyLane tally_load(const double* row, bool all) {
    const int l = lane_id();
    const bool hdr = (l >= 32) & (l < 40);
    TallyLane t{0.0, 0.0};
    if ((l < 25) | hdr | ((l >= 40) & all)) {
        const int w = tally_word(l);
        t.a = row[w];
        t.b = row[hdr ? (((TALLY_SUM_LANES >> (l - 32)) & 1u) ? 2 : 3) : w + 1];
    }
    return t;
}
DEV void tally_store(double* row, const TallyLane& t, float rew, const i32 (&iw)[HFTLOB_INFO_AGENT_WORDS], u32 f32,
                     bool all) {
    const int l = lane_id();
    const int k = l < 25 ? l - 1 : l - 40;
    i32 v = 0;
#pragma unroll
    for (int j = 0; j < HFTLOB_INFO_AGENT_WORDS; ++j) v = k == j ? iw[j] : v;
    double x = ((f32 >> (k & 31)) & 1u) ? (double)bitf(v) : (double)v;
    if (l == 0) x = (double)rew;
    if ((l >= 32) & (l < 40)) {
        const int h = l - 32;
        const double run = t.b + (((TALLY_SUM_LANES >> h) & 1u) ? (double)rew : 1.0);
        double a;
        if (h == 0) a = t.a + 1.0;
        else if (h == 1) a = t.a + (all ? 1.0 : 0.0);
        else if (h < 4) a = all ? 0.0 : run;
        else if ((h & 1) == 0) a = all ? t.a + run : t.a;
        else a = all ? t.a + run * run : t.a;
        row[h] = a;
    } else if ((l < 25) | ((l >= 40) & all)) {
        const int w = tally_word(l);
        row[w] = t.a + x;
        row[w + 1] = t.b + x * x;
    }
}
template <int S, int NFIX, bool RC, bool RA = false, bool QUIET = false, int PK = -1, bool TALLY = false,
          int BAKED = -1>
DEV bool env_step_dev(const hftlob_env_cfg& c_rt, int key_n, int ek, int e, const u32* __restrict__ keys, bool master,
                      Key& mk,
                      i32* __restrict__ actions_io, const i32* __restrict__ msg_data,
                      const i32* __restrict__ init_states, i32* __restrict__ state, float* __restrict__ obs_out,
                      float* __restrict__ rew_out, u8* __restrict__ done_all_out, u8* __restrict__ dones_out,
                      i32* __restrict__ info_out, i32* __restrict__ obs_raw_out, i32* __restrict__ msgs_out,
                      i32* __restrict__ debug_out, i32* lds, bool resident, bool keep, u32& fl_carry,
                      const i32* pre_keys = nullptr, bool emit_rt = true, double* __restrict__ stats = nullptr,
                      int act_e = -1) {
    const hftlob_env_cfg& c = baked_cfg<BAKED>(c_rt);
    constexpr int UNR = baked_unroll<BAKED>();
    const bool emit = !QUIET && emit_rt;
    const bool vals = TALLY || emit;
    STAMP(t_start);
#ifdef HFTLOB_STAMPS
    const unsigned long long rt_start = __builtin_amdgcn_s_memrealtime();
#endif
    const int l = lane_id();
    const int M = c.n_msgs, D = c.n_data_msg, A = c.n_action_msgs, C = c.n_cancel_msgs;
    i32* rec = state + (size_t)e * c.rec_words;
    Book<S> B;
    B.c = lobcfg(c.lob);
    if (NFIX > 0) { B.c.nO = NFIX; B.c.nT = NFIX; }
    const int R = B.c.nO;
    const LdsMap LM = lds_map(c, B.c.nO, B.c.nT, RA);
    i32* rows = lds + LM.rows;
    i32* axs = lds + LM.axs;
    book_bind(B, lds + LM.book);
    SideRows<S> fa, fb;
    if (!resident) {
        fetch_side(fa, rec + c.off_asks, B.vs);
        fetch_side(fb, rec + c.off_bids, B.vs);
    }
    const int naw = c.rec_words - c.off_agents;
    const bool agw_pre = naw <= 64;
    const i32 agw = (agw_pre & (l < naw)) ? rec[c.off_agents + l] : 0;
    const bool batched = PK == 1 || (PK < 0 && pre_keys);
    const StepKeys SK = batched ? load_keys(c, pre_keys) : step_keys<NFIX == 0>(c, key_n, ek, keys, master, mk);
    if (master && !batched) mk = SK.next_master;
    const Key key_reset = SK.key_reset;
    if (RC) {
        B.ek = c.shuffle_action_messages ? split_key(SK.k1, 2, 0, c.prng_partitionable) : SK.k1;
        B.nmsg = M;
        B.part = c.prng_partitionable;
    }
    SUBSTAMP(t_keys);
    const i32* Lr = rec + c.off_loaded;
    const i32* Wr = rec + c.off_world;
    const i32 ld_t0 = Lr[LD_T0], win = Lr[LD_WIN], max_steps = Lr[LD_MAXS], start_index = Lr[LD_START],
              step = Lr[LD_STEP];
    const i32 wt0 = Wr[W_T0], wt1 = Wr[W_T1], oidc = Wr[W_OIDC];
    const float wmid = bitf(Wr[W_MID]);
    const i32 old_last_ba = rec[c.off_best_asks + (M - 1) * 2], old_last_bb = rec[c.off_best_bids + (M - 1) * 2];
    bool excl_any = false, excl_cfg = false;
#pragma unroll UNR
    for (int t = 0; t < c.n_types; ++t) {
        const bool ex = c.types[t].kind == HFTLOB_AGENT_MM && c.types[t].exclude_extreme_spreads;
        excl_cfg |= ex;
        if (vals && ex) {
            bool any = false;
            for (int m = l; m < M; m += 64) {
                const i32 pa = rec[c.off_best_asks + m * 2], pb = rec[c.off_best_bids + m * 2];
                any |= (i2f(wsub(pa, pb)) / (i2f(wadd(pa, pb)) / 2.0f)) > 0.1f;
            }
            excl_any = ballot(any) != 0ull;
        }
    }
    const bool store_best = NFIX == 0 || (!keep | excl_cfg);
    i32 dstart = wadd(start_index, wmul(D, step));
    dstart = imax_(0, imin_(dstart, c_rt.n_data_rows - D));
    const bool ftime = NFIX == 0 && c.ep_type == 1;
    const i32 t_end = wadd(ld_t0, c.episode_time);
    int4 px = make_int4(0, 0, 0, 0), py = px;
    if ((l >= C + A) & (l < M)) {
        const i32* g = msg_data + (size_t)(dstart + l - (C + A)) * 8;
        ld_msg(g, px, py);
        if (ftime) fixed_time_mask(px, py, t_end);
    }
    if (resident) {
        relink_side(B.a, R, B.vs);
        relink_side(B.b, R, B.vs);
        B.fl = fl_carry | F_STALE_A | F_STALE_B | STALE_ANY;
    } else {
        B.fl = commit_side<true>(B.a, fa, R, B.vs) | commit_side<false>(B.b, fb, R, B.vs) | F_STALE_A | F_STALE_B | STALE_ANY;
        B.fl |= slow_bit(B.fl);
    }
    SUBSTAMP(t_load);

#ifdef HFTLOB_STAMPS
    unsigned long long acc_act = 0, acc_cnl = 0, acc_flt = 0, acc_mmr = 0, acc_exr = 0, acc_obs = 0;
#endif
    constexpr bool REG = NFIX > 0 && !RA;
    RegRows<S> sink;
    if constexpr (REG) {
        SUBSTAMP(tc0);
        sink.init(B.a.t, B.b.t, R, C, wt0, wt1);
        STAMP_ACC(acc_cnl, tc0);
    }
    const auto srows = row_sink<REG>(sink, rows);
    {
        int ag = 0, arow = C, crow = 0, aw = 0;
        const i32* st = rec + c.off_agents;
#pragma unroll UNR
        for (int t = 0; t < c.n_types; ++t) {
            const hftlob_agent_type_cfg& tc = c.types[t];
#pragma unroll UNR
            for (int i = 0; i < tc.n_agents; ++i, ++ag) {
                const i32 tid = wsub(tc.trader_id0, i);
                const int w = tc.action_width;
                i32* aio = actions_io ? actions_io + (size_t)(act_e < 0 ? e : act_e) * c.action_words + aw : nullptr;
                aw += w;
                i32 act, av[4] = {0, 0, 0, 0};
                if (NFIX > 0 || w == 1) {
                    if (master) {
                        act = rdl(SK.acts, 32 + ag);
                        if (aio && l == 0) aio[0] = act;
                    } else {
                        act = aio[0];
                    }
                    av[0] = act;
                } else {
                    i32 v = 0;
                    if (master) {
                        const bool part = c.prng_partitionable;
                        const Key ka = split_key(split_key(SK.key, c.n_types, t, part), tc.n_agents, i, part);
                        v = randint_vec(ka, w, l < w ? l : 0, 0, action_hi(tc), part);
                        if (aio && l < w) aio[l] = v;
                    } else if (l < w) {
                        v = aio[l];
                    }
#pragma unroll
                    for (int j = 0; j < 4; ++j) av[j] = rdl(v, j);
                    act = av[0];
                }
                i32 s4[4];
                {
                    const int b = (int)(st - (rec + c.off_agents));
#pragma unroll
                    for (int k = 0; k < 4; ++k) s4[k] = agw_pre ? rdl(agw, b + k) : st[k];
                }
                ActX x{0, 0, 0, 0, 0, 0};
                SUBSTAMP(ta0);
#if defined(HFTLOB_KO_ACT) || defined(HFTLOB_KO_CNL)
                for (int k = 0; k < tc.n_msgs; ++k) {
#ifndef HFTLOB_KO_ACT
                    if (k < tc.n_action_msgs) continue;
#endif
#ifndef HFTLOB_KO_CNL
                    if (k >= tc.n_action_msgs) continue;
#endif
                    put_row(srows, k < tc.n_action_msgs ? arow + k : crow + k - tc.n_action_msgs, 0, 0, 0, 0, 0, 0, 0, 0);
                }
#endif
#ifdef HFTLOB_DUP_AGENT
                i32 z_ = 0;
                asm volatile("s_mov_b32 %0, 0" : "=s"(z_));
                for (int rep = 0; rep < 2; ++rep) {
                const i32 tid_r = tid ^ (rep * z_), act_r = act ^ (rep * z_), ba_r = old_last_ba ^ (rep * z_);
                const bool do_act = rep == 0 || (HFTLOB_DUP_AGENT & 1), do_cnl = rep == 0 || (HFTLOB_DUP_AGENT & 2);
#else
                {
                const i32 tid_r = tid, act_r = act, ba_r = old_last_ba;
                constexpr bool do_act = true, do_cnl = true;
#endif
                if (tc.kind == HFTLOB_AGENT_MM) {
#ifndef HFTLOB_KO_ACT
                    if (!do_act) {
                    } else if (tc.action_space == HFTLOB_MM_ACT_DIRECTIONAL)
                        mm_directional(c, tc, tid_r, act_r, wt0, wt1, ba_r, old_last_bb, srows, arow, x);
                    else if (tc.action_space == HFTLOB_MM_ACT_FIXED_QUANTS)
                        mm_fixed_quant(c, tc, B, s4, tid_r, act_r, wt0, wt1, ba_r, old_last_bb, srows, arow, x);
                    else
                        mm_other_actions(c, tc, B, s4, tid_r, act_r, wt0, wt1, ba_r, old_last_bb, step, ld_t0, srows,
                                         arow, x);
#endif
                    STAMP_ACC(acc_act, ta0);
                    SUBSTAMP(ta1);
                    const int sz = tc.n_msgs / 4;
#ifndef HFTLOB_KO_CNL
                    if constexpr (REG) {
                        if (do_cnl) {
                            cancel_regs(sink, sink.bt, sink.bq, sink.bo, B.b.pc, B.vs, tid_r, sz, 1, crow);
                            cancel_regs(sink, sink.at, sink.aq, sink.ao, B.a.pc, B.vs, tid_r, sz, -1, crow + sz);
                        }
                    } else if (do_cnl) {
                        cancel_rows(B.b, R, B.vs, tid_r, sz, 1, wt0, wt1, rows, crow);
                        cancel_rows(B.a, R, B.vs, tid_r, sz, -1, wt0, wt1, rows, crow + sz);
                    }
#endif
                    STAMP_ACC(acc_cnl, ta1);
                } else {
#ifndef HFTLOB_KO_ACT
                    if (!do_act) {
                    } else if (NFIX == 0 && tc.action_space == HFTLOB_EXE_ACT_FIXED_PRICES)
                        exe_fixed_prices(c, tc, rec, s4, tid_r, av, wt0, wt1, srows, arow);
                    else
                        exe_fqc(c, tc, s4, tid_r, act_r, wt0, wt1, ba_r, old_last_bb, step, max_steps, srows, arow);
#endif
                    STAMP_ACC(acc_act, ta0);
                    SUBSTAMP(ta1);
#ifndef HFTLOB_KO_CNL
                    const i32 sell = s4[3];
                    if constexpr (REG) {
                        if (do_cnl) {
                            if (sell) cancel_regs(sink, sink.at, sink.aq, sink.ao, B.a.pc, B.vs, tid_r, tc.n_msgs / 2, -1, crow);
                            else cancel_regs(sink, sink.bt, sink.bq, sink.bo, B.b.pc, B.vs, tid_r, tc.n_msgs / 2, 1, crow);
                        }
                    } else if (do_cnl) {
                        cancel_rows(sell ? B.a : B.b, R, B.vs, tid_r, tc.n_msgs / 2, wsub(1, wmul(sell, 2)), wt0, wt1,
                                    rows, crow);
                    }
#endif
                    STAMP_ACC(acc_cnl, ta1);
                }
                }
                SUBSTAMP(ta2);
                {
                    const i32 xv[6] = {x.bid_price, x.ask_price, x.bid_dist, x.ask_dist, x.bid_quant, x.ask_quant};
                    i32 v = 0;
#pragma unroll
                    for (int k = 0; k < 6; ++k) if (l == k) v = xv[k];
                    if (l < 6) axs[ag * 6 + l] = v;
                }
                if constexpr (REG)
                    sink.agent(arow, crow, tc.n_action_msgs, tid, wadd(wt0, tc.time_delay_obs_act),
                               wadd(wt1, tc.time_delay_obs_act));
#ifndef HFTLOB_KO_FILTER
                if constexpr (!REG) {
                    if (tc.n_action_msgs == 2) filter_rows<2>(rows, arow, crow, B.a.scr);
                    else if (tc.n_action_msgs == 4) filter_rows<4>(rows, arow, crow, B.a.scr);
                    else if (NFIX == 0 && tc.n_action_msgs == 3) filter_rows<3>(rows, arow, crow, B.a.scr);
                    else filter_rows<1>(rows, arow, crow, B.a.scr);
                }
#endif
                STAMP_ACC(acc_flt, ta2);
                arow += tc.n_action_msgs;
                crow += tc.n_msgs - tc.n_action_msgs;
                st += agent_words(tc);
            }
        }
    }
#ifndef HFTLOB_KO_FILTER
    if constexpr (REG) {
        SUBSTAMP(tf0);
        filter_regs(sink, C);
        STAMP_ACC(acc_flt, tf0);
    }
#endif
    wave_sync();
    SUBSTAMP(t_rows);
    if constexpr (REG) {
        const int j = l - C;
        const bool act_lane = (j >= 0) & (j < A);
        if (act_lane) sink.y.x = wsub(oidc, j);
        if (c.shuffle_action_messages && A >= 2) {
            const u32 bits = (u32)__builtin_amdgcn_ds_bpermute((j & 63) << 2, (i32)SK.shuffle_bits);
            int rank = 0;
            for (int k = 0; k < A; ++k) {
                const u32 bk = (u32)rdl((i32)SK.shuffle_bits, k);
                rank += (bk < bits) || (bk == bits && k < j);
            }
            const int dest = (act_lane ? C + rank : l) << 2;
            sink.x.x = __builtin_amdgcn_ds_permute(dest, sink.x.x); sink.x.y = __builtin_amdgcn_ds_permute(dest, sink.x.y);
            sink.x.z = __builtin_amdgcn_ds_permute(dest, sink.x.z); sink.x.w = __builtin_amdgcn_ds_permute(dest, sink.x.w);
            sink.y.x = __builtin_amdgcn_ds_permute(dest, sink.y.x); sink.y.y = __builtin_amdgcn_ds_permute(dest, sink.y.y);
            sink.y.z = __builtin_amdgcn_ds_permute(dest, sink.y.z); sink.y.w = __builtin_amdgcn_ds_permute(dest, sink.y.w);
        }
    } else {
        i32 f[8];
        const bool act_lane = l < A;
        if (act_lane) {
#pragma unroll
            for (int k = 0; k < 8; ++k) f[k] = rows[(C + l) * 8 + k];
            f[4] = wsub(oidc, l);
        }
        int dest = l;
        if (c.shuffle_action_messages && A >= 2) {
            const u32 bits = SK.shuffle_bits;
            int rank = 0;
            for (int j = 0; j < A; ++j) {
                const u32 bj = (u32)rdl((i32)bits, j);
                rank += (bj < bits) || (bj == bits && j < l);
            }
            dest = rank;
        }
        wave_sync();
        if (act_lane) {
#pragma unroll
            for (int k = 0; k < 8; ++k) rows[(C + dest) * 8 + k] = f[k];
        }
        wave_sync();
    }

    STAMP(t_agents);
    if (!RA) trades_fill(B.tr, B.vt, -1);
    B.ntr = 0;
    const int AR = C + A;
    bool abort_any = false;
    i32 prev_a = -1, prev_b = -1;
    float mid_acc = 0.0f, pa_acc = 0.0f, pb_acc = 0.0f;
    i32 last_p_a = 0, last_p_b = 0, last_t0 = 0, last_t1 = 0;
    int4 nx = px, ny = py;
    if constexpr (REG) {
        if (l < AR) { nx = sink.x; ny = sink.y; }
    }
#ifndef HFTLOB_NO_CARRY
    i32* carry = B.filt - PAD_FILT + PAD_CARRY;
    if (!RA && resident) {
        const i32 v = carry[l & 15];
        B.a.best_p = rdl(v, 0); B.a.best_q = rdl(v, 1); B.a.xp = rdl(v, 2); B.a.top = rdl(v, 3);
        B.a.top_p = rdl(v, 4); B.a.top_ts = rdl(v, 5); B.a.top_tns = rdl(v, 6);
        B.b.best_p = rdl(v, 7); B.b.best_q = rdl(v, 8); B.b.top = rdl(v, 9); B.b.top_p = rdl(v, 10);
        B.b.top_ts = rdl(v, 11); B.b.top_tns = rdl(v, 12);
        B.fl &= ~(F_STALE_A | F_STALE_B | STALE_ANY);
    }
#endif
#ifdef HFTLOB_STAMPS_CHUNK
    unsigned long long acc_dec = 0, acc_pre = 0, acc_loop = 0, acc_post = 0;
#endif
    for (int base = 0; base < M; base += 64) {
#ifdef HFTLOB_STAMPS_CHUNK
        const unsigned long long tc0 = __builtin_amdgcn_s_memtime();
#endif
        const int row = base + l;
        int4 x = nx, y = ny;
        if (REG) {
        } else if (RA ? (base == 0) & (row < AR) : row < AR) {
            x = reinterpret_cast<const int4*>(rows + row * 8)[0];
            y = reinterpret_cast<const int4*>(rows + row * 8)[1];
        } else if (ftime && base > 0 && row >= AR) {
            fixed_time_mask(x, y, t_end);
        }
        if (msgs_out && row < M) {
            int4* mo = reinterpret_cast<int4*>(msgs_out + ((size_t)e * M + row) * 8);
            mo[0] = x;
            mo[1] = y;
        }
        {
            const bool nv = (row + 64 >= AR) & (row + 64 < M);
            ld_msg(msg_data + (size_t)(dstart + (nv ? row + 64 - AR : 0)) * 8, nx, ny);
        }
        if (RA && (base == 0)) {
            if (row + 64 < AR) {
                nx = reinterpret_cast<const int4*>(rows + (row + 64) * 8)[0];
                ny = reinterpret_cast<const int4*>(rows + (row + 64) * 8)[1];
            }
            wave_sync();
            trades_fill(B.tr, B.vt, -1);
        }
        decode_msgs(B.c, x, y);
        i32 rpa = 0, rqa = 0, rpb = 0, rqb = 0;
        const int cnt = uni(imin_(64, M - base));
#ifdef HFTLOB_STAMPS_CHUNK
        acc_dec += __builtin_amdgcn_s_memtime() - tc0;
#endif
        run_chunk<RC>(B, x, y, cnt, base, rpa, rqa, rpb, rqb CHUNK_ARGS);
#ifdef HFTLOB_STAMPS_CHUNK
        const unsigned long long tc1 = __builtin_amdgcn_s_memtime();
#endif
        abort_any |= bal((l < cnt) & ((rpa == -1) | (rpb == -1))) != 0ull;
        i32 pa = rpa, pb = rpb;
        if ((base == 0) & (l == 0)) {
            pa = pa == -1 ? old_last_ba : pa;
            pb = pb == -1 ? old_last_bb : pb;
        }
        const i32 caq = rpa == -1 ? 0 : rqa, cbq = rpb == -1 ? 0 : rqb;
        const i32 cap = ffill(pa, prev_a), cbp = ffill(pb, prev_b);
        prev_a = rdl(cap, cnt - 1);
        prev_b = rdl(cbp, cnt - 1);
        if ((row < M) & (store_best | (row == M - 1))) {
            reinterpret_cast<int2*>(rec + c.off_best_asks)[row] = make_int2(cap, caq);
            reinterpret_cast<int2*>(rec + c.off_best_bids)[row] = make_int2(cbp, cbq);
        }
        if (row < M) {
            const float mf = i2f(wadd(cbp, cap)) / 2.0f;
            mid_acc = base == 0 ? mf : mid_acc + mf;
            if (info_out) {
                pa_acc = base == 0 ? i2f(cap) : pa_acc + i2f(cap);
                pb_acc = base == 0 ? i2f(cbp) : pb_acc + i2f(cbp);
            }
        }
        if (base + 64 >= M) {
            last_t0 = rdl(y.z, cnt - 1);
            last_t1 = rdl(y.w, cnt - 1);
        }
#ifdef HFTLOB_STAMPS_CHUNK
        acc_post += __builtin_amdgcn_s_memtime() - tc1;
#endif
    }
    last_p_a = prev_a;
    last_p_b = prev_b;
#ifndef HFTLOB_NO_CARRY
    if (!RA && keep) {
        i32 v = B.a.best_p;
        v = wlane(v, B.a.best_q, 1); v = wlane(v, B.a.xp, 2); v = wlane(v, B.a.top, 3); v = wlane(v, B.a.top_p, 4);
        v = wlane(v, B.a.top_ts, 5); v = wlane(v, B.a.top_tns, 6); v = wlane(v, B.b.best_p, 7);
        v = wlane(v, B.b.best_q, 8); v = wlane(v, B.b.top, 9); v = wlane(v, B.b.top_p, 10);
        v = wlane(v, B.b.top_ts, 11); v = wlane(v, B.b.top_tns, 12);
        if (l < 13) carry[l] = v;
    }
#endif
    StepCtx X;
    X.avg_mid = wave_fsum(mid_acc) / (float)M;
    X.last_ba = last_p_a; X.last_bb = last_p_b;
    X.last_mid = i2f(wadd(last_p_b, last_p_a)) / 2.0f;
    X.wmid = wmid;
    X.old_last_ba = old_last_ba; X.old_last_bb = old_last_bb;
    X.init0 = ld_t0; X.step = step;
    X.ep_done = wsub(wsub(max_steps, step), 1) <= 1;
    const bool all = X.ep_done;

    STAMP(t_book);
    WorldView wv;
    wv.best_ask_p = last_p_a; wv.best_bid_p = last_p_b;
    wv.vol_a = wv.vol_b = 0;
    if (emit) { wv.vol_a = side_volume(B.a, R, B.vs); wv.vol_b = side_volume(B.b, R, B.vs); }
    if (debug_out) write_debug(B, debug_out + (size_t)e * HFTLOB_DEBUG_WORDS(B.c.nT));
    if (keep) fl_carry = B.fl;
    if (!all & !keep) {
        store_side(B.a, rec + c.off_asks, R, B.vs);
        store_side(B.b, rec + c.off_bids, R, B.vs);
        store_trades(B.tr, rec + c.off_trades, B.vt);
    }
    wv.step = wadd(step, 1); wv.max_steps = max_steps; wv.mid = X.last_mid;
    wv.t0 = last_t0; wv.t1 = last_t1; wv.it0 = ld_t0; wv.it1 = Lr[LD_T1];
    const float dt = i2f(last_t0) + i2f(last_t1) / 1e9f - i2f(wt0) - i2f(wt1) / 1e9f;
    wv.dt = dt;
    i32* info = info_out ? info_out + (size_t)e * c.info_words : nullptr;
    if (vals | !all) {
        TradeView<S> TV;
        {
            const i32 ovr0[8] = {0, 0, 0, 0, 0, 0, 0, 0};
            trade_view(B, TV, false, -1, ovr0);
        }
        int ag = 0;
        i32* st = rec + c.off_agents;
#pragma unroll UNR
        for (int t = 0; t < c.n_types; ++t) {
            const hftlob_agent_type_cfg& tc = c.types[t];
#pragma unroll UNR
            for (int i = 0; i < tc.n_agents; ++i, ++ag) {
                const i32 tid = wsub(tc.trader_id0, i);
                const int nw = agent_words(tc);
                i32 s[13];
                {
                    const int b = (int)(st - (rec + c.off_agents));
                    for (int k = 0; k < 13; ++k) s[k] = k < nw ? (agw_pre ? rdl(agw, b + k) : st[k]) : 0;
                }
                i32 d = 0;
                float rew;
                TallyLane tl{0.0, 0.0};
#ifndef HFTLOB_KO_TALLY
                if constexpr (TALLY) tl = tally_load(stats + ((size_t)e * c.n_agents + ag) * HFTLOB_EVAL_WORDS, all);
#endif
                i32 iw[HFTLOB_INFO_AGENT_WORDS];
                for (int k = 0; k < HFTLOB_INFO_AGENT_WORDS; ++k) iw[k] = 0;
                ActX ax1;
                ax1.bid_price = uni(axs[ag * 6 + 0]); ax1.ask_price = uni(axs[ag * 6 + 1]);
                ax1.bid_dist = uni(axs[ag * 6 + 2]); ax1.ask_dist = uni(axs[ag * 6 + 3]);
                ax1.bid_quant = uni(axs[ag * 6 + 4]); ax1.ask_quant = uni(axs[ag * 6 + 5]);
                SUBSTAMP(tr0);
                if (tc.kind == HFTLOB_AGENT_MM) {
                    MMRew R;
#if defined(HFTLOB_KO_REWARD) || defined(HFTLOB_KO_MM_REWARD)
                    memset(&R, 0, sizeof R);
#else
                    mm_reward(c, tc, B, X, s, tid, excl_any, TV, R, vals);
#endif
                    STAMP_ACC(acc_mmr, tr0);
                    const float tot = bitf(s[3]) + R.PnL;
                    s[0] = ax1.bid_dist; s[1] = ax1.ask_dist; s[2] = R.end_inventory; s[3] = fbit(tot);
                    s[4] = fbit(R.cash);
                    rew = R.reward / tc.reward_scaling_quo;
                    iw[0] = fbit(R.reward); iw[1] = fbit(R.reward_pv); iw[2] = fbit(R.reward_spooner);
                    iw[3] = fbit(R.end_of_ep_pv); iw[4] = fbit(R.reward_spooner_damped);
                    iw[5] = fbit(R.reward_spooner_asym_damped); iw[6] = fbit(R.reward_spooner_asym_damped2);
                    iw[7] = fbit(R.reward_delta_pv); iw[8] = fbit(tot); iw[9] = 0; iw[10] = s[2];
                    iw[11] = fbit(R.delta_mid); iw[12] = fbit(R.market_share); iw[13] = fbit(R.buyPnL);
                    iw[14] = R.forced_unwind; iw[15] = fbit(R.invPnL); iw[16] = ax1.bid_price;
                    iw[17] = ax1.ask_price; iw[18] = ax1.bid_dist; iw[19] = ax1.ask_dist;
                    iw[20] = ax1.ask_quant; iw[21] = ax1.bid_quant; iw[22] = fbit(R.sellPnL);
                    iw[23] = fbit(R.inventoryValue);
                } else {
                    EXRew R;
#if defined(HFTLOB_KO_REWARD) || defined(HFTLOB_KO_EXE_REWARD)
                    memset(&R, 0, sizeof R);
#else
                    exe_reward(c, tc, B, X, s, tid, TV, R, vals);
#endif
                    STAMP_ACC(acc_exr, tr0);
                    s[2] = wadd(s[2], R.agentQuant);
                    s[4] = fbit(R.p_vwap);
                    s[5] = fbit(bitf(s[5]) + i2f(R.qp_agent));
                    s[6] = fbit(bitf(s[6]) + R.drift);
                    s[7] = fbit(bitf(s[7]) + R.advantage);
                    s[8] = fbit(R.slippage_rm); s[9] = fbit(R.price_adv_rm); s[10] = fbit(R.price_drift_rm);
                    s[11] = fbit(R.vwap_rm); s[12] = fbit(R.trade_duration);
                    d = wsub(s[1], s[2]) <= 0;
                    rew = R.reward / tc.reward_scaling_quo;
                    iw[0] = R.quant_left; iw[1] = d; iw[2] = fbit(R.slippage); iw[3] = fbit(R.vwap_rm);
                    iw[4] = fbit(R.drift); iw[5] = fbit(R.advantage); iw[6] = R.doom_quant; iw[7] = s[3];
                    iw[8] = fbit(R.reward_info);
                }
#ifndef HFTLOB_KO_TALLY
                if constexpr (TALLY)
                    tally_store(stats + ((size_t)e * c.n_agents + ag) * HFTLOB_EVAL_WORDS, tl, rew, iw,
                                tc.kind == HFTLOB_AGENT_MM ? INFO_F32_MM : INFO_F32_EXE, all);
#endif
                if (emit & (l == 0)) {
                    rew_out[(size_t)e * c.n_agents + ag] = rew;
                    dones_out[(size_t)e * c.n_agents + ag] = (u8)(d != 0);
                }
                if (info) {
                    i32 v = 0;
                    for (int k = 0; k < HFTLOB_INFO_AGENT_WORDS; ++k) if (l == k) v = iw[k];
                    if (l < HFTLOB_INFO_AGENT_WORDS) info[HFTLOB_INFO_WORLD_WORDS + ag * HFTLOB_INFO_AGENT_WORDS + l] = v;
                }
                SUBSTAMP(to0);
                if (!all) {
                    i32 v = 0;
                    for (int k = 0; k < 13; ++k) if (l == k) v = s[k];
                    if (l < nw) st[l] = v;
#ifndef HFTLOB_KO_OBS
                    if (emit)
                        write_obs<false>(c, tc, wv, s, obs_out + ((size_t)e * c.n_agents + ag) * c.obs_stride, d != 0,
                                         ftime);
#endif
                }
                if (obs_raw_out)
                    write_obs<true>(c, tc, wv, s, obs_raw_out + ((size_t)e * c.n_agents + ag) * c.obs_stride, false,
                                    ftime);
                STAMP_ACC(acc_obs, to0);
                st += nw;
            }
        }
    }
    STAMP(t_rewards);
    const float new_mid = X.last_mid;
    if (info) {
        const float ava = wave_fsum(pa_acc) / (float)M, avb = wave_fsum(pb_acc) / (float)M;
        i32 wv_[HFTLOB_INFO_WORLD_WORDS] = {win, fbit(new_mid), wadd(step, 1), last_t0, last_t1, wsub(oidc, A),
                                            last_p_a, last_p_b, fbit(ava), fbit(avb), fbit(dt), (i32)X.ep_done,
                                            (i32)abort_any, wsub(last_p_a, last_p_b)};
        i32 v = 0;
        for (int k = 0; k < HFTLOB_INFO_WORLD_WORDS; ++k) if (l == k) v = wv_[k];
        if (l < HFTLOB_INFO_WORLD_WORDS) info[l] = v;
    }
    if (emit & (l == 0)) done_all_out[e] = (u8)all;
#ifdef HFTLOB_STAMPS
    if (info && l == 0) {
        const unsigned long long t_end = __builtin_amdgcn_s_memtime();
        info[0] = (i32)(t_agents - t_start); info[1] = (i32)(t_book - t_agents);
        info[2] = (i32)(t_rewards - t_book); info[3] = (i32)(t_end - t_rewards); info[4] = (i32)all;
#ifndef HFTLOB_STAMPS_COARSE
        info[5] = (i32)(t_keys - t_start); info[6] = (i32)(t_load - t_keys); info[7] = (i32)(t_rows - t_load);
        info[8] = (i32)(t_agents - t_rows);
#else
        info[5] = info[6] = info[7] = info[8] = 0;
        (void)t_keys; (void)t_load; (void)t_rows;
#endif
#ifdef HFTLOB_STAMPS_CHUNK
        info[9] = (i32)acc_dec; info[10] = (i32)acc_pre; info[11] = (i32)acc_loop; info[12] = (i32)acc_post;
        info[13] = 0; info[14] = 0;
        (void)acc_act; (void)acc_cnl; (void)acc_flt; (void)acc_mmr; (void)acc_exr; (void)acc_obs;
#else
        info[9] = (i32)acc_act; info[10] = (i32)acc_cnl; info[11] = (i32)acc_flt;
        info[12] = (i32)acc_mmr; info[13] = (i32)acc_exr; info[14] = (i32)acc_obs;
#endif
        info[15] = (i32)(__builtin_amdgcn_s_memrealtime() - rt_start);
    }
#endif
    if (all) {
        env_reset_dev<S, BAKED>(c_rt, key_reset, init_states, rec,
                                emit ? obs_out + (size_t)e * c.n_agents * c.obs_stride : nullptr, B.vs, B.vt, ftime);
        return true;
    }
    if (l == 0) {
        rec[c.off_loaded + LD_STEP] = wadd(step, 1);
        i32* W = rec + c.off_world;
        W[W_T0] = last_t0; W[W_T1] = last_t1; W[W_OIDC] = wsub(oidc, A); W[W_MID] = fbit(new_mid); W[W_DT] = fbit(dt);
    }
    return false;
}

template <int S, int NFIX, bool RC, bool RA = false>
__global__ __launch_bounds__(64) void k_env_step(hftlob_env_cfg c, int n_env, int key_e0, int key_n,
                                                 const u32* __restrict__ keys, const u32* __restrict__ master,
                                                 u32* __restrict__ master_out, i32* __restrict__ actions_io,
                                                 const i32* __restrict__ msg_data, const i32* __restrict__ init_states,
                                                 i32* __restrict__ state, hftlob_step_out out) {
    one_wave();
    extern __shared__ __attribute__((aligned(16))) i32 lds[];
    const int e = blockIdx.x;
    if (e >= n_env) return;
    Key mk{0u, 0u};
    if (master) mk = Key{master[0], master[1]};
    u32 fl = 0;
    env_step_dev<S, NFIX, RC, RA>(c, key_n, key_e0 + e, e, keys, master != nullptr, mk, actions_io, msg_data, init_states,
                              state, out.obs, out.rewards, out.done_all, out.dones, out.info, out.obs_raw, out.msgs,
                              out.debug, lds, false, false, fl);
    if (master && (e == 0) && (lane_id() == 0)) { master_out[0] = mk.a; master_out[1] = mk.b; }
}

typedef const __attribute__((address_space(4))) hftlob_env_cfg kcfg_t;

#define WAVE_SLOTS (8 * 16 * 16 * 64)
static __device__ unsigned long long g_wave_eta[WAVE_SLOTS];
DEV unsigned long long* wave_row(u32 hwid, u32 xcc, u32& slot) {
    const u32 cu = ((xcc & 7u) * 16u + ((hwid >> 13) & 7u) * 2u + ((hwid >> 12) & 1u)) * 16u + ((hwid >> 8) & 15u);
    slot = ((hwid >> 4) & 3u) * 16u + (hwid & 15u);
    return g_wave_eta + (size_t)cu * 64u;
}
#ifndef HFTLOB_PRIO_SCOPE
#define HFTLOB_PRIO_SCOPE __HIP_MEMORY_SCOPE_WORKGROUP
#endif
DEV void balance_prio(unsigned long long* row, u32 slot, unsigned long long r0, int done, int left) {
    const int l = lane_id();
    const unsigned long long now = __builtin_amdgcn_s_memrealtime();
    const float el = (float)(now - r0);
    const unsigned long long eta = now + (unsigned long long)(el * ((float)left / (float)done));
    if (l == 0) __hip_atomic_store(row + slot, eta, __ATOMIC_RELAXED, HFTLOB_PRIO_SCOPE);
    unsigned long long v = __hip_atomic_load(row + l, __ATOMIC_RELAXED, HFTLOB_PRIO_SCOPE);
    v = (u32)l == slot ? eta : v;
    v = ((u32)l >> 4) == (slot >> 4) ? v : 0ull;
    const lmask live = bal(v > now);
    const lmask later = live & bal((v > eta) | ((v == eta) & ((u32)l < slot)));
    const int n = __builtin_popcountll(live), rank = __builtin_popcountll(later);
    const int q = n > 0 ? (4 * rank) / n : 0;
    if (q == 0) __builtin_amdgcn_s_setprio(3);
    else if (q == 1) __builtin_amdgcn_s_setprio(2);
    else if (q == 2) __builtin_amdgcn_s_setprio(1);
    else __builtin_amdgcn_s_setprio(0);
}
template <int S, int NFIX, bool RC, bool RA = false, int KB = -1, int BAKED = -1>
__global__ __launch_bounds__(64, 4) void k_env_rollout(hftlob_env_cfg c_arg, int n_env, int key_e0, int key_n, int n_steps,
                                                    int per_step, const u32* __restrict__ master,
                                                    u32* __restrict__ master_out, i32* __restrict__ actions_io,
                                                    const i32* __restrict__ msg_data,
                                                    const i32* __restrict__ init_states, i32* __restrict__ state,
                                                    hftlob_step_out out) {
    one_wave();
    extern __shared__ __attribute__((aligned(16))) i32 lds[];
    const int e = blockIdx.x;
    if (e >= n_env) return;
    Key mk{master[0], master[1]};
    kcfg_t* kp = (kcfg_t*)__builtin_amdgcn_kernarg_segment_ptr();
    bool resident = false;
    u32 fl = 0;
#ifndef HFTLOB_NO_BALANCE
    const unsigned long long bal_r0 = __builtin_amdgcn_s_memrealtime();
    const u32 bal_hwid = __builtin_amdgcn_s_getreg(0xF804), bal_xcc = __builtin_amdgcn_s_getreg(0x7814);
    u32 bal_slot;
    unsigned long long* bal_row = wave_row(bal_hwid, bal_xcc, bal_slot);
#endif
#ifdef HFTLOB_WAVETIME
    const unsigned long long wt_start = __builtin_amdgcn_s_memtime(), wt_rstart = __builtin_amdgcn_s_memrealtime();
    const u32 wt_hwid = __builtin_amdgcn_s_getreg(0xF804), wt_xcc = __builtin_amdgcn_s_getreg(0x7814);
#endif
    const hftlob_env_cfg& c = baked_cfg<BAKED>(c_arg);
    const bool kbat = KB < 0 ? kb_ok(c) : KB == 1;
    const int kbw = kb_words(c);
    i32* kbuf = lds + lds_map(c, NFIX > 0 ? NFIX : c.lob.n_orders, NFIX > 0 ? NFIX : c.lob.n_trades, RA).kb;
    auto step = [&](auto Q, int t) {
        constexpr bool QT = decltype(Q)::value;
        const size_t o = per_step ? (size_t)t * n_env : 0;
        const int tb = t % KB_STEPS;
        kcfg_t* cp = kp;
        i32* st = state;
        const i32* md = msg_data;
        const i32* is = init_states;
        asm volatile("" : "+s"(cp), "+s"(st), "+s"(md), "+s"(is));
        const hftlob_env_cfg& cr = *(const hftlob_env_cfg*)cp;
        const hftlob_env_cfg& cc = baked_cfg<BAKED>(cr);
        STAMP(kb0);
        if (kbat && tb == 0) step_keys_batch<NFIX == 0>(cc, key_n, key_e0 + e, mk, imin_(KB_STEPS, n_steps - t), kbuf);
        STAMP(kb1);
        const bool ox = !QT;
#ifdef HFTLOB_STAMPS_QUIET
        const bool ox_info = true;
#else
        const bool ox_info = ox;
#endif
        const bool reset = env_step_dev<S, NFIX, RC, RA, QT, KB, false, BAKED>(
            cr, key_n, key_e0 + e, e, nullptr, true, mk, actions_io ? actions_io + o * cc.action_words : nullptr, md,
            is, st, out.obs + o * cc.n_agents * cc.obs_stride, out.rewards + o * cc.n_agents, out.done_all + o,
            out.dones + o * cc.n_agents, ox_info && out.info ? out.info + o * cc.info_words : nullptr,
            ox && out.obs_raw ? out.obs_raw + o * cc.n_agents * cc.obs_stride : nullptr,
            ox && out.msgs ? out.msgs + o * cc.n_msgs * 8 : nullptr,
            ox && out.debug ? out.debug + o * (size_t)HFTLOB_DEBUG_WORDS(cc.lob.n_trades) : nullptr, lds,
            NFIX > 0 && resident, NFIX > 0 && t + 1 < n_steps, fl, kbat ? kbuf + tb * kbw : nullptr, !QT);
        resident = uni(!reset) != 0;
        STAMP(bp0);
#ifndef HFTLOB_NO_BALANCE
#ifndef HFTLOB_BALANCE_EVERY
#define HFTLOB_BALANCE_EVERY 1
#endif
#ifndef HFTLOB_BALANCE_MIN_ENVS
#define HFTLOB_BALANCE_MIN_ENVS 1024
#endif
        if ((t + 1 < n_steps) && ((t % HFTLOB_BALANCE_EVERY) == 0) && (n_env > HFTLOB_BALANCE_MIN_ENVS))
            balance_prio(bal_row, bal_slot, bal_r0, t + 1, n_steps - t - 1);
#endif
#ifdef HFTLOB_STAMPS
        if (out.info && per_step && lane_id() == 0) {
            i32* irow = out.info + ((size_t)t * n_env + e) * cc.info_words;
            irow[16] = (i32)(kb1 - kb0);
            irow[17] = (i32)(__builtin_amdgcn_s_memtime() - bp0);
        }
#endif
#ifdef HFTLOB_WAVETIME
        if (out.info && per_step) {
            const unsigned long long now = __builtin_amdgcn_s_memtime(), rnow = __builtin_amdgcn_s_memrealtime();
            const i32 w10[10] = {(i32)(u32)now, (i32)(u32)(now >> 32), (i32)wt_hwid, (i32)wt_xcc, (i32)(u32)wt_start,
                                 (i32)(u32)(wt_start >> 32), (i32)(u32)rnow, (i32)(u32)(rnow >> 32),
                                 (i32)(u32)wt_rstart, (i32)(u32)(wt_rstart >> 32)};
            i32 v = 0;
#pragma unroll
            for (int k = 0; k < 10; ++k) v = lane_id() == k ? w10[k] : v;
            if (lane_id() < 10) out.info[((size_t)t * n_env + e) * cc.info_words + lane_id()] = v;
        }
#endif
    };
    int t = 0;
#ifdef HFTLOB_STAMPS_QUIET
    if (true) {
#else
    if (!per_step) {
#endif
#pragma unroll 1
        for (; t + 1 < n_steps; ++t) step(std::integral_constant<bool, true>{}, t);
    }
#pragma unroll 1
    for (; t < n_steps; ++t) step(std::integral_constant<bool, false>{}, t);
#ifndef HFTLOB_NO_BALANCE
    if (lane_id() == 0) __hip_atomic_store(bal_row + bal_slot, __builtin_amdgcn_s_memrealtime(), __ATOMIC_RELAXED,
                                           HFTLOB_PRIO_SCOPE);
#endif
    if ((e == 0) && (lane_id() == 0)) { master_out[0] = mk.a; master_out[1] = mk.b; }
}

template <int S, int NFIX, bool RC, bool RA = false>
__global__ __launch_bounds__(64, 4) void k_env_rollout_actions(hftlob_env_cfg c, int n_env, int n_steps, int per_step,
                                                            const u32* __restrict__ keys,
                                                            const i32* __restrict__ actions,
                                                            const i32* __restrict__ msg_data,
                                                            const i32* __restrict__ init_states,
                                                            i32* __restrict__ state, hftlob_step_out out) {
    one_wave();
    extern __shared__ __attribute__((aligned(16))) i32 lds[];
    const int e = blockIdx.x;
    if (e >= n_env) return;
    Key mk{0u, 0u};
    kcfg_t* kp = (kcfg_t*)__builtin_amdgcn_kernarg_segment_ptr();
    bool resident = false;
    u32 fl = 0;
#ifndef HFTLOB_NO_BALANCE
    const unsigned long long bal_r0 = __builtin_amdgcn_s_memrealtime();
    const u32 bal_hwid = __builtin_amdgcn_s_getreg(0xF804), bal_xcc = __builtin_amdgcn_s_getreg(0x7814);
    u32 bal_slot;
    unsigned long long* bal_row = wave_row(bal_hwid, bal_xcc, bal_slot);
#endif
    auto step = [&](auto Q, int t) {
        constexpr bool QT = decltype(Q)::value;
        const size_t o = per_step ? (size_t)t * n_env : 0;
        kcfg_t* cp = kp;
        i32* st = state;
        const i32* md = msg_data;
        const i32* is = init_states;
        asm volatile("" : "+s"(cp), "+s"(st), "+s"(md), "+s"(is));
        const hftlob_env_cfg& cc = *(const hftlob_env_cfg*)cp;
        const bool ox = !QT;
        const bool reset = env_step_dev<S, NFIX, RC, RA, QT, 0>(
            cc, n_env, e, e, keys + (size_t)t * n_env * 2, false, mk,
            const_cast<i32*>(actions) + (size_t)t * n_env * cc.action_words, md, is, st,
            out.obs + o * cc.n_agents * cc.obs_stride, out.rewards + o * cc.n_agents, out.done_all + o,
            out.dones + o * cc.n_agents, ox && out.info ? out.info + o * cc.info_words : nullptr,
            ox && out.obs_raw ? out.obs_raw + o * cc.n_agents * cc.obs_stride : nullptr,
            ox && out.msgs ? out.msgs + o * cc.n_msgs * 8 : nullptr,
            ox && out.debug ? out.debug + o * (size_t)HFTLOB_DEBUG_WORDS(cc.lob.n_trades) : nullptr, lds,
            NFIX > 0 && resident, NFIX > 0 && t + 1 < n_steps, fl, nullptr, !QT);
        resident = uni(!reset) != 0;
#ifndef HFTLOB_NO_BALANCE
        if ((t + 1 < n_steps) && ((t % HFTLOB_BALANCE_EVERY) == 0) && (n_env > HFTLOB_BALANCE_MIN_ENVS))
            balance_prio(bal_row, bal_slot, bal_r0, t + 1, n_steps - t - 1);
#endif
    };
    int t = 0;
    if (!per_step) {
#pragma unroll 1
        for (; t + 1 < n_steps; ++t) step(std::integral_constant<bool, true>{}, t);
    }
#pragma unroll 1
    for (; t < n_steps; ++t) step(std::integral_constant<bool, false>{}, t);
#ifndef HFTLOB_NO_BALANCE
    if (lane_id() == 0) __hip_atomic_store(bal_row + bal_slot, __builtin_amdgcn_s_memrealtime(), __ATOMIC_RELAXED,
                                           HFTLOB_PRIO_SCOPE);
#endif
}

template <int S, int NFIX, bool RC, bool RA = false>
__global__ __launch_bounds__(64, 4) void k_env_rollout_eval(hftlob_env_cfg c, int n_env, int n_steps, int fixed,
                                                         const u32* __restrict__ keys,
                                                         const i32* __restrict__ actions,
                                                         const i32* __restrict__ msg_data,
                                                         const i32* __restrict__ init_states,
                                                         i32* __restrict__ state, double* __restrict__ stats,
                                                         hftlob_step_out out) {
    one_wave();
    extern __shared__ __attribute__((aligned(16))) i32 lds[];
    const int e = blockIdx.x;
    if (e >= n_env) return;
    Key mk{0u, 0u};
    kcfg_t* kp = (kcfg_t*)__builtin_amdgcn_kernarg_segment_ptr();
    bool resident = false;
    u32 fl = 0;
#ifndef HFTLOB_NO_BALANCE
    const unsigned long long bal_r0 = __builtin_amdgcn_s_memrealtime();
    const u32 bal_hwid = __builtin_amdgcn_s_getreg(0xF804), bal_xcc = __builtin_amdgcn_s_getreg(0x7814);
    u32 bal_slot;
    unsigned long long* bal_row = wave_row(bal_hwid, bal_xcc, bal_slot);
#endif
    auto step = [&](auto Q, int t) {
        constexpr bool QT = decltype(Q)::value;
        kcfg_t* cp = kp;
        i32* st = state;
        const i32* md = msg_data;
        const i32* is = init_states;
        double* sp = stats;
        asm volatile("" : "+s"(cp), "+s"(st), "+s"(md), "+s"(is), "+s"(sp));
        const hftlob_env_cfg& cc = *(const hftlob_env_cfg*)cp;
        const bool ox = !QT;
        const bool reset = env_step_dev<S, NFIX, RC, RA, QT, 0, true>(
            cc, n_env, e, e, keys + (size_t)t * n_env * 2, false, mk,
            const_cast<i32*>(actions) + (fixed ? (size_t)0 : (size_t)t * n_env * cc.action_words), md, is, st, out.obs,
            out.rewards, out.done_all, out.dones, ox ? out.info : nullptr, ox ? out.obs_raw : nullptr,
            ox ? out.msgs : nullptr, ox ? out.debug : nullptr, lds, NFIX > 0 && resident, NFIX > 0 && t + 1 < n_steps, fl,
            nullptr, !QT, sp, fixed ? 0 : -1);
        resident = uni(!reset) != 0;
#ifndef HFTLOB_NO_BALANCE
        if ((t + 1 < n_steps) && ((t % HFTLOB_BALANCE_EVERY) == 0) && (n_env > HFTLOB_BALANCE_MIN_ENVS))
            balance_prio(bal_row, bal_slot, bal_r0, t + 1, n_steps - t - 1);
#endif
    };
    int t = 0;
#pragma unroll 1
    for (; t + 1 < n_steps; ++t) step(std::integral_constant<bool, true>{}, t);
    step(std::integral_constant<bool, false>{}, t);
#ifndef HFTLOB_NO_BALANCE
    if (lane_id() == 0) __hip_atomic_store(bal_row + bal_slot, __builtin_amdgcn_s_memrealtime(), __ATOMIC_RELAXED,
                                           HFTLOB_PRIO_SCOPE);
#endif
}

#if !defined(HFTLOB_INST)
__global__ void k_sample_actions(hftlob_env_cfg c, int n_env, const u32* __restrict__ keys, i32* __restrict__ actions) {
    const int e = blockIdx.x * blockDim.x + threadIdx.x;
    if (e >= n_env) return;
    const bool part = c.prng_partitionable;
    const Key k{keys[2 * e], keys[2 * e + 1]};
    i32* out = actions + (size_t)e * c.action_words;
    for (int t = 0; t < c.n_types; ++t) {
        const hftlob_agent_type_cfg& tc = c.types[t];
        const Key sub = split_key(k, c.n_types, t, part);
        const int w = tc.action_width;
        const i32 hi = action_hi(tc);
        for (int i = 0; i < tc.n_agents; ++i) {
// ... 610 lines not shown
```

Measured before the change: 102.4 million.

## Add lazy best-quantity mode that skips best-level quantity tracking in quiet kernels

Adds an LZ template path, enabled for quiet kernels with fixed agents, no RA, and no extreme-spread exclusion. In that path the book's best-level quantity is no longer tracked. Rescans compute only the best price and skip loading the quantity column, and per-message recording writes only the price. When a reduced order is cleared, the code checks via a ballot whether its price level is now empty instead of decrementing a quantity. Per-row best-quantity stores are dropped except for the final row, and a carry flag forces a full rescan when a non-lazy kernel resumes after a lazy one. This trades per-message reductions, bpermutes and global stores for extra correctness complexity around the carried state.

```diff
diff --git a/jaxmarl-hft_amd/csrc/hftlob.hip b/jaxmarl-hft_amd/csrc/hftlob.hip
--- a/jaxmarl-hft_amd/csrc/hftlob.hip
+++ b/jaxmarl-hft_amd/csrc/hftlob.hip
@@ -312,11 +312,17 @@
     i32 top, top_p, top_ts, top_tns;
     i32 rp, rq;
     lmask rm;
+#ifdef HFTLOB_STAMPS_CHUNK
+    u32 n_resc, n_rec;
+#endif
 };
-template <int S> DEV void side_rec(Side<S>& s, u32 k) {
+template <bool LZ = false, int S> DEV void side_rec(Side<S>& s, u32 k) {
     s.rp = wlane(s.rp, s.best_p, (int)k);
-    s.rq = wlane(s.rq, s.best_q, (int)k);
+    if (!LZ) s.rq = wlane(s.rq, s.best_q, (int)k);
     asm volatile("s_bitset1_b64 %0, %1" : "+s"(s.rm) : "s"(k));
+#ifdef HFTLOB_STAMPS_CHUNK
+    ++s.n_rec;
+#endif
 }
 
 template <int S> DEV void col_set(i32 (&c)[S], int e, i32 v) {
@@ -326,7 +332,7 @@
 }
 
 enum : u32 { F_STALE_A = 2, F_STALE_B = 4, F_CLEAN_A = 8, F_CLEAN_B = 16, F_NEG1_A = 32, F_NEG1_B = 64,
-             F_PM1_A = 256, F_PM1_B = 512, F_STALE_ANY = 0x40000000u, F_SLOW = 0x80000000u };
+             F_PM1_A = 256, F_PM1_B = 512, F_LAZY = 0x20000000u, F_STALE_ANY = 0x40000000u, F_SLOW = 0x80000000u };
 constexpr u32 STALE_ANY = F_STALE_ANY;
 template <bool ASKS> struct SideBits {
     static constexpr u32 STALE = ASKS ? F_STALE_A : F_STALE_B;
@@ -458,14 +464,36 @@
     bp = pa;
     bq = wave_sum(v);
 }
-template <bool ASKS, bool REC, int S>
+template <int S> DEV i32 best_bid_p(const i32 (&p)[S], const Valid<S>& V) {
+    i32 m = INT_MIN;
+#pragma unroll
+    for (int r = 0; r < S; ++r) m = imax_(m, V.v[r] ? p[r] : INT_MIN);
+    return wave_max(m);
+}
+template <int S> DEV i32 best_ask_p(const i32 (&p)[S], const Valid<S>& V, i32 maxint, i32& xp) {
+    i32 m = INT_MAX;
+#pragma unroll
+    for (int r = 0; r < S; ++r) m = imin_(m, V.v[r] ? (p[r] == -1 ? maxint : p[r]) : INT_MAX);
+    const i32 mn = wave_min(m);
+    xp = mn;
+    return mn == maxint ? -1 : mn;
+}
+template <bool ASKS, bool REC, bool LZ = false, int S>
 DEV void rescan(Side<S>& s, u32& fl, int R, const Valid<S>& V, i32 maxint, u32 k) {
-    i32 q[S];
-    ldcol(s.t, R, FQ, q);
-    if (ASKS) best_ask_pq(s.pc, q, V, maxint, s.best_p, s.best_q, &s.xp);
-    else best_bid_pq(s.pc, q, V, s.best_p, s.best_q);
+    if (LZ) {
+        if (ASKS) s.best_p = best_ask_p(s.pc, V, maxint, s.xp);
+        else s.best_p = best_bid_p(s.pc, V);
+    } else {
+        i32 q[S];
+        ldcol(s.t, R, FQ, q);
+        if (ASKS) best_ask_pq(s.pc, q, V, maxint, s.best_p, s.best_q, &s.xp);
+        else best_bid_pq(s.pc, q, V, s.best_p, s.best_q);
+    }
     fl &= ~SideBits<ASKS>::STALE;
-    if (REC) side_rec(s, k);
+    if (REC) side_rec<LZ>(s, k);
+#ifdef HFTLOB_STAMPS_CHUNK
+    ++s.n_resc;
+#endif
 }
 
 template <int S>
@@ -593,7 +621,7 @@
     }
 }
 #define XP_SET(s, v) ((s).xp = (v))
-template <bool BID, int S, bool STALE_OK = true, bool NN = false>
+template <bool BID, int S, bool STALE_OK = true, bool NN = false, bool LZ = false>
 DEV void note_add(Side<S>& s, u32& fl, int e, i32 np, i32 nq, i32 t, i32 tns, i32 maxint, u32 k) {
     constexpr u32 STALE = SideBits<!BID>::STALE, MARK = SideBits<!BID>::MARK;
     if (STALE_OK && (fl & STALE)) { s.top = -1; return; }
@@ -602,51 +630,59 @@
         if (np < bp) {
             if (!NN && bp == -1) fl |= MARK;
         } else if (np > bp) {
-            s.best_p = np; s.best_q = nq;
-            side_rec(s, k);
+            s.best_p = np;
+            if (!LZ) s.best_q = nq;
+            side_rec<LZ>(s, k);
             top_new(s, e, np, t, tns, maxint);
         } else if (!NN && bp == -1) {
             fl |= MARK;
         } else {
-            s.best_q = wadd(s.best_q, nq);
-            side_rec(s, k);
+            if (!LZ) { s.best_q = wadd(s.best_q, nq); side_rec(s, k); }
             top_eq(s, e, t, tns, maxint);
         }
     } else if (NN && !STALE_OK) {
         const i32 xp = s.xp;
         if (np > xp) {
         } else if (np < xp) {
-            s.best_p = np; s.best_q = nq; XP_SET(s, np); side_rec(s, k); top_new(s, e, np, t, tns, maxint);
+            s.best_p = np; if (!LZ) s.best_q = nq; XP_SET(s, np); side_rec<LZ>(s, k); top_new(s, e, np, t, tns, maxint);
         } else if (np == maxint) {
             fl |= MARK;
         } else {
-            s.best_q = wadd(s.best_q, nq);
-            side_rec(s, k);
+            if (!LZ) { s.best_q = wadd(s.best_q, nq); side_rec(s, k); }
             top_eq(s, e, t, tns, maxint);
         }
     } else {
         if (np > bp) {
             if (bp == -1) {
                 if (np == maxint) fl |= MARK;
-                else { s.best_p = np; s.best_q = nq; XP_SET(s, np); side_rec(s, k); top_new(s, e, np, t, tns, maxint); }
+                else { s.best_p = np; if (!LZ) s.best_q = nq; XP_SET(s, np); side_rec<LZ>(s, k); top_new(s, e, np, t, tns, maxint); }
             }
         } else if (np < bp) {
-            if (NN || np != -1) { s.best_p = np; s.best_q = nq; XP_SET(s, np); side_rec(s, k); top_new(s, e, np, t, tns, maxint); }
+            if (NN || np != -1) { s.best_p = np; if (!LZ) s.best_q = nq; XP_SET(s, np); side_rec<LZ>(s, k); top_new(s, e, np, t, tns, maxint); }
         } else if (!NN && np == -1) {
             fl |= MARK;
         } else if (np != maxint) {
-            s.best_q = wadd(s.best_q, nq);
-            side_rec(s, k);
+            if (!LZ) { s.best_q = wadd(s.best_q, nq); side_rec(s, k); }
             top_eq(s, e, t, tns, maxint);
         }
     }
 }
-template <bool ASKS, int S> DEV void note_reduce(Side<S>& s, u32& fl, i32 op, i32 dq, u32 k) {
+template <bool ASKS, bool LZ = false, bool G = false, int S>
+DEV void note_reduce(Side<S>& s, u32& fl, i32 op, i32 dq, u32 k, bool cleared) {
     constexpr u32 STALE = SideBits<ASKS>::STALE, MARK = SideBits<ASKS>::MARK;
     if (fl & STALE) return;
     if (op == s.best_p) {
         if (op == -1) {
             fl |= MARK;
+        } else if (LZ) {
+            if (G) {
+                fl |= MARK;
+            } else if (cleared) {
+                lmask at = 0;
+#pragma unroll
+                for (int r = 0; r < S; ++r) at |= bal(s.pc[r] == op);
+                if (at == 0ull) fl |= MARK;
+            }
         } else {
             s.best_q = wsub(s.best_q, dq);
             side_rec(s, k);
@@ -682,7 +718,7 @@
     return a == 0ull;
 }
 
-template <bool G, bool ASKS, int S>
+template <bool G, bool ASKS, bool LZ = false, int S>
 DEV i32 match_order(Book<S>& B, Side<S>& s, int top, i32 qtm, const Msg& m, i32 qt, i32 pt, i32 ot, i32 tt) {
     const int R = B.c.nO;
     const i32 newq = imax_(0, wsub(qt, qtm));
@@ -703,7 +739,7 @@
     if (!G || (B.fl & SideBits<ASKS>::CLEAN)) {
         if (newq <= 0) side_clr(s, R, top);
         else stu(s.t, s.scr, R, FQ, top, newq);
-        note_reduce<ASKS>(s, B.fl, pt, wsub(qt, newq), m.k);
+        note_reduce<ASKS, LZ, G>(s, B.fl, pt, wsub(qt, newq), m.k, newq <= 0);
     } else {
         stu(s.t, s.scr, R, FQ, top, newq);
         rzn<ASKS>(s, B.fl, R, B.vs);
@@ -711,7 +747,7 @@
     return rem;
 }
 
-template <bool BID, bool G, int S, bool POS = false>
+template <bool BID, bool G, int S, bool POS = false, bool LZ = false>
 DEV i32 match_against(Book<S>& B, Side<S>& s, i32 qtm, i32 price, const Msg& m) {
     const int R = B.c.nO;
     if (!POS && fresh(qtm) <= 0) return qtm;
@@ -721,7 +757,7 @@
         if (__builtin_expect(BID ? mp0 < price : mp0 > price, 1)) return qtm;
     }
     while (qtm > 0) {
-        if (B.fl & SideBits<!BID>::STALE) rescan<!BID, true>(s, B.fl, R, B.vs, B.c.maxint, m.k);
+        if (B.fl & SideBits<!BID>::STALE) rescan<!BID, true, LZ>(s, B.fl, R, B.vs, B.c.maxint, m.k);
         i32 mp = s.best_p;
         if (!BID) {
             if (mp == -1) {
@@ -752,12 +788,12 @@
         if (fresh(tp) == -1) break;
         asm volatile("");
         if (BID ? tp < price : tp > price) break;
-        qtm = match_order<G, !BID>(B, s, top, qtm, m, qt, tp, ot, tt);
+        qtm = match_order<G, !BID, LZ>(B, s, top, qtm, m, qt, tp, ot, tt);
     }
     return qtm;
 }
 
-template <bool BID, bool G, int S>
+template <bool BID, bool G, bool LZ = false, int S>
 DEV void add_order(Book<S>& B, Side<S>& s, const Msg& m, i32 qty, const lmask (&free)[S]) {
     const int R = B.c.nO;
     constexpr u32 CLEAN = SideBits<!BID>::CLEAN, NEG1 = SideBits<!BID>::NEG1, MARK = SideBits<!BID>::MARK,
@@ -769,7 +805,7 @@
         if (nq > 0) {
             side_put(s, R, e, m.price, nq, m.oid, m.tid, m.t, m.tns);
             if (m.h & (H_NEG1 | H_PM1)) B.fl = B.fl | (m.h & H_NEG1 ? NEG1 : 0u) | (m.h & H_PM1 ? PM1 : 0u) | F_SLOW;
-            if (was_empty) note_add<BID>(s, B.fl, e, m.price, nq, m.t, m.tns, B.c.maxint, m.k);
+            if (was_empty) note_add<BID, S, true, false, LZ>(s, B.fl, e, m.price, nq, m.t, m.tns, B.c.maxint, m.k);
             else { B.fl |= MARK; s.top = -1; }
         } else if (!was_empty) {
             side_clr(s, R, e);
@@ -805,7 +841,7 @@
         side_put(s, R, e, m.price, nq, m.oid, m.tid, m.t, m.tns);
         if (m.h & H_NEG1) B.fl |= NEG1;
         if (m.h & H_PM1) B.fl |= PM1;
-        if (was_empty) note_add<BID>(s, B.fl, e, m.price, nq, m.t, m.tns, B.c.maxint, m.k);
+        if (was_empty) note_add<BID, S, true, false, LZ>(s, B.fl, e, m.price, nq, m.t, m.tns, B.c.maxint, m.k);
         else { B.fl |= MARK; s.top = -1; }
     } else if (!was_empty) {
         side_clr(s, R, e);
@@ -834,7 +870,7 @@
 #pragma unroll
     for (int r = 0; r < S; ++r) free[r] = m[r];
 }
-template <bool BID, bool RARE, int S, bool POS = false>
+template <bool BID, bool RARE, int S, bool POS = false, bool LZ = false>
 DEV void add_free(Book<S>& B, Side<S>& s, const Msg& m, i32 qty, const lmask (&free)[S]) {
     const int R = B.c.nO;
     if (!POS && qty <= 0) return;
@@ -860,71 +896,71 @@
         constexpr u32 NEG1 = SideBits<!BID>::NEG1, PM1 = SideBits<!BID>::PM1;
         B.fl = B.fl | (m.h & H_NEG1 ? NEG1 : 0u) | (m.h & H_PM1 ? PM1 : 0u) | F_SLOW;
     }
-    note_add<BID, S, false, !RARE>(s, B.fl, (int)e, m.price, qty, m.t, m.tns, B.c.maxint, m.k);
-}
-template <bool BID, int S> DEV bool add_common(Book<S>& B, Side<S>& s, const Msg& m, const lmask (&free)[S]) {
+    note_add<BID, S, false, !RARE, LZ>(s, B.fl, (int)e, m.price, qty, m.t, m.tns, B.c.maxint, m.k);
+}
+template <bool BID, bool LZ = false, int S> DEV bool add_common(Book<S>& B, Side<S>& s, const Msg& m, const lmask (&free)[S]) {
 #ifndef HFTLOB_OLD_ADD_TEST
     if (S == 2) {
         if (__builtin_expect(free[0] != 0ull, 1)) {
-            add_free<BID, false, S, true>(B, s, m, m.qty, free);
+            add_free<BID, false, S, true, LZ>(B, s, m, m.qty, free);
             return true;
         }
         if (free[S - 1] == 0ull) return false;
-        add_free<BID, false, S, true>(B, s, m, m.qty, free);
+        add_free<BID, false, S, true, LZ>(B, s, m, m.qty, free);
         return true;
     }
 #endif
     if (no_slot(free)) return false;
-    add_free<BID, false, S, true>(B, s, m, m.qty, free);
+    add_free<BID, false, S, true, LZ>(B, s, m, m.qty, free);
     return true;
 }
-template <bool G, bool RARE, int S> DEV void bid_lim(Book<S>& B, Msg m) {
+template <bool G, bool RARE, bool LZ = false, int S> DEV void bid_lim(Book<S>& B, Msg m) {
     if (!RARE) __builtin_assume(m.qty > 0);
     constexpr bool POS = !RARE && !G;
     if (POS) {
         if (__builtin_expect(B.a.xp > m.price, 1)) {
             lmask free[S];
             free_slots(B, B.b, free);
-            if (add_common<true>(B, B.b, m, free)) return;
+            if (add_common<true, LZ>(B, B.b, m, free)) return;
             if (B.c.check_fill) evict_if_full<true>(B, B.b, free);
-            add_order<true, G>(B, B.b, m, m.qty, free);
+            add_order<true, G, LZ>(B, B.b, m, m.qty, free);
             return;
         }
     }
-    const i32 rem = match_against<false, G, S, POS>(B, B.a, m.qty, m.price, m);
+    const i32 rem = match_against<false, G, S, POS, LZ>(B, B.a, m.qty, m.price, m);
     if (RARE && __builtin_expect((m.h & H_MKT) != 0, 0)) m.price = B.c.maxint;
     lmask free[S];
     free_slots(B, B.b, free);
     if (!no_slot(free)) {
-        if (!G) add_free<true, RARE>(B, B.b, m, (RARE && (m.h & H_DISCARD)) ? 0 : rem, free);
-        else if (!(m.h & H_DISCARD)) add_order<true, G>(B, B.b, m, rem, free);
+        if (!G) add_free<true, RARE, S, false, LZ>(B, B.b, m, (RARE && (m.h & H_DISCARD)) ? 0 : rem, free);
+        else if (!(m.h & H_DISCARD)) add_order<true, G, LZ>(B, B.b, m, rem, free);
         return;
     }
     if (B.c.check_fill) evict_if_full<true>(B, B.b, free);
-    if (!(m.h & H_DISCARD)) add_order<true, G>(B, B.b, m, rem, free);
-}
-template <bool G, bool RARE, int S> DEV void ask_lim(Book<S>& B, Msg m) {
+    if (!(m.h & H_DISCARD)) add_order<true, G, LZ>(B, B.b, m, rem, free);
+}
+template <bool G, bool RARE, bool LZ = false, int S> DEV void ask_lim(Book<S>& B, Msg m) {
     if (!RARE) __builtin_assume(m.qty > 0);
     if (RARE && __builtin_expect((m.h & H_MKT) != 0, 0)) m.price = 0;
     constexpr bool POS = !RARE && !G;
     if (POS && __builtin_expect(B.b.best_p < m.price, 1)) {
         lmask free[S];
         free_slots(B, B.a, free);
-        if (add_common<false>(B, B.a, m, free)) return;
+        if (add_common<false, LZ>(B, B.a, m, free)) return;
         if (B.c.check_fill) evict_if_full<false>(B, B.a, free);
-        add_order<false, G>(B, B.a, m, m.qty, free);
+        add_order<false, G, LZ>(B, B.a, m, m.qty, free);
         return;
     }
-    const i32 rem = match_against<true, G, S, POS>(B, B.b, m.qty, m.price, m);
+    const i32 rem = match_against<true, G, S, POS, LZ>(B, B.b, m.qty, m.price, m);
     lmask free[S];
     free_slots(B, B.a, free);
     if (!no_slot(free)) {
-        if (!G) add_free<false, RARE>(B, B.a, m, (RARE && (m.h & H_DISCARD)) ? 0 : rem, free);
-        else if (!(m.h & H_DISCARD)) add_order<false, G>(B, B.a, m, rem, free);
+        if (!G) add_free<false, RARE, S, false, LZ>(B, B.a, m, (RARE && (m.h & H_DISCARD)) ? 0 : rem, free);
+        else if (!(m.h & H_DISCARD)) add_order<false, G, LZ>(B, B.a, m, rem, free);
         return;
     }
     if (B.c.check_fill) evict_if_full<false>(B, B.a, free);
-    if (!(m.h & H_DISCARD)) add_order<false, G>(B, B.a, m, rem, free);
+    if (!(m.h & H_DISCARD)) add_order<false, G, LZ>(B, B.a, m, rem, free);
 }
 template <int S>
 DEV int random_id_match(const Book<S>& B, Key& k, const i32 (&o)[S], const lmask (&pm)[S]) {
@@ -958,7 +994,7 @@
     for (int r = 0; r < S; ++r) f[r] = B.vs.m[r] & bal(o[r] == chosen);
     return first_slot(f, -1);
 }
-template <bool G, bool ASKS, bool RC, int S> DEV void cancel(Book<S>& B, Side<S>& s, const Msg& m) {
+template <bool G, bool ASKS, bool RC, bool LZ = false, int S> DEV void cancel(Book<S>& B, Side<S>& s, const Msg& m) {
     if (!G && m.qty == 0) return;
     const int R = B.c.nO;
     int idx;
@@ -1029,7 +1065,7 @@
     if (!G || (B.fl & SideBits<ASKS>::CLEAN)) {
         if (nq <= 0) side_clr(s, R, idx);
         else stu(s.t, s.scr, R, FQ, idx, nq);
-        note_reduce<ASKS>(s, B.fl, op, wsub(oq, nq > 0 ? nq : 0), m.k);
+        note_reduce<ASKS, LZ, G>(s, B.fl, op, wsub(oq, nq > 0 ? nq : 0), m.k, nq <= 0);
     } else {
         stu(s.t, s.scr, R, FQ, idx, nq);
         rzn<ASKS>(s, B.fl, R, B.vs);
@@ -1056,29 +1092,29 @@
     x.x = h;
     x.y = sd;
 }
-template <bool G, bool RC, int S>
+template <bool G, bool RC, bool LZ = false, int S>
 DEV void process_msg_(Book<S>& B, u32 k, i32 h, i32 sdv, i32 d2, i32 d3, i32 d4, i32 d5, i32 d6, i32 d7) {
     Msg m;
     m.h = h; m.side = 0; m.price = d3; m.qty = d2; m.oid = d4; m.tid = d5; m.t = d6; m.tns = d7;
     m.k = k;
     const i32 kind = h & H_KIND;
-    if (kind == H_CNL_ASK) cancel<G, true, RC>(B, B.a, m);
-    else if (kind == H_CNL_BID) cancel<G, false, RC>(B, B.b, m);
+    if (kind == H_CNL_ASK) cancel<G, true, RC, LZ>(B, B.a, m);
+    else if (kind == H_CNL_BID) cancel<G, false, RC, LZ>(B, B.b, m);
     else if (kind == H_BID) {
         if (!G && !(h & H_RARE)) {
             m.side = 1;
-            bid_lim<G, false>(B, m);
+            bid_lim<G, false, LZ>(B, m);
         } else {
             m.side = rdl(sdv, k);
-            bid_lim<G, true>(B, m);
+            bid_lim<G, true, LZ>(B, m);
         }
     } else if (kind == H_ASK) {
         if (!G && !(h & H_RARE)) {
             m.side = -1;
-            ask_lim<G, false>(B, m);
+            ask_lim<G, false, LZ>(B, m);
         } else {
             m.side = rdl(sdv, k);
-            ask_lim<G, true>(B, m);
+            ask_lim<G, true, LZ>(B, m);
         }
     }
 }
@@ -1090,10 +1126,10 @@
     const i32 got = __builtin_amdgcn_ds_bpermute(src << 2, v);
     return src < 0 ? carry : got;
 }
-template <bool REC = true, int S> DEV void refresh_best(Book<S>& B, u32 k = 0) {
+template <bool REC = true, bool LZ = false, int S> DEV void refresh_best(Book<S>& B, u32 k = 0) {
     if (B.fl & STALE_ANY) {
-        if (B.fl & F_STALE_A) rescan<true, REC>(B.a, B.fl, B.c.nO, B.vs, B.c.maxint, k);
-        if (B.fl & F_STALE_B) rescan<false, REC>(B.b, B.fl, B.c.nO, B.vs, B.c.maxint, k);
+        if (B.fl & F_STALE_A) rescan<true, REC, LZ>(B.a, B.fl, B.c.nO, B.vs, B.c.maxint, k);
+        if (B.fl & F_STALE_B) rescan<false, REC, LZ>(B.b, B.fl, B.c.nO, B.vs, B.c.maxint, k);
         B.fl &= ~STALE_ANY;
     }
 }
@@ -1184,7 +1220,7 @@
 #define CHUNK_PARAMS
 #define CHUNK_ARGS
 #endif
-template <bool RC, int S>
+template <bool RC, bool LZ = false, int S>
 DEV void run_chunk(Book<S>& B, const int4& x, const int4& y, int cnt, int base, i32& rpa, i32& rqa, i32& rpb,
                    i32& rqb CHUNK_PARAMS) {
 #ifdef HFTLOB_STAMPS_CHUNK
@@ -1203,10 +1239,11 @@
 #ifdef HFTLOB_KO_LOOP
     todo = 0;
 #endif
-    refresh_best<false>(B);
-    const i32 cpa = B.a.best_p, cqa = B.a.best_q, cpb = B.b.best_p, cqb = B.b.best_q;
+    refresh_best<false, LZ>(B);
+    const i32 cpa = B.a.best_p, cqa = LZ ? 0 : B.a.best_q, cpb = B.b.best_p, cqb = LZ ? 0 : B.b.best_q;
     B.a.rm = B.b.rm = 0ull;
-    B.a.rp = B.a.rq = B.b.rp = B.b.rq = 0;
+    B.a.rp = B.b.rp = 0;
+    if (!LZ) B.a.rq = B.b.rq = 0;
 #ifdef HFTLOB_STAMPS_CHUNK
     const unsigned long long tp1 = __builtin_amdgcn_s_memtime();
     acc_pre += tp1 - tp0;
@@ -1218,9 +1255,9 @@
         do {
             asm volatile("s_bitset0_b64 %0, %1" : "+s"(todo) : "s"(k));
             if (RC) B.mi = base + (int)k;
-            if ((i32)B.fl >= 0) process_msg_<false, RC>(B, k, h, x.y, d2, d3, d4, d5, d6, d7);
-            else process_msg_<true, RC>(B, k, h, x.y, d2, d3, d4, d5, d6, d7);
-            refresh_best(B, k);
+            if ((i32)B.fl >= 0) process_msg_<false, RC, LZ>(B, k, h, x.y, d2, d3, d4, d5, d6, d7);
+            else process_msg_<true, RC, LZ>(B, k, h, x.y, d2, d3, d4, d5, d6, d7);
+            refresh_best<true, LZ>(B, k);
             const u32 kn = ff1(todo);
             h = rdl(hx, kn); d2 = rdl(x.z, kn); d3 = rdl(x.w, kn);
             d4 = rdl(y.x, kn); d5 = rdl(y.y, kn); d6 = rdl(y.z, kn); d7 = rdl(y.w, kn);
@@ -1235,8 +1272,8 @@
         const lmask below = ~0ull >> (63 - l);
         const lmask ma = B.a.rm & below, mb = B.b.rm & below;
         const int sa = ma ? 63 - __builtin_clzll(ma) : -1, sb = mb ? 63 - __builtin_clzll(mb) : -1;
-        const i32 gpa = __builtin_amdgcn_ds_bpermute(sa << 2, B.a.rp), gqa = __builtin_amdgcn_ds_bpermute(sa << 2, B.a.rq);
-        const i32 gpb = __builtin_amdgcn_ds_bpermute(sb << 2, B.b.rp), gqb = __builtin_amdgcn_ds_bpermute(sb << 2, B.b.rq);
+        const i32 gpa = __builtin_amdgcn_ds_bpermute(sa << 2, B.a.rp), gqa = LZ ? 0 : __builtin_amdgcn_ds_bpermute(sa << 2, B.a.rq);
+        const i32 gpb = __builtin_amdgcn_ds_bpermute(sb << 2, B.b.rp), gqb = LZ ? 0 : __builtin_amdgcn_ds_bpermute(sb << 2, B.b.rq);
         rpa = sa < 0 ? cpa : gpa;
         rqa = sa < 0 ? cqa : gqa;
         rpb = sb < 0 ? cpb : gpb;
@@ -1251,6 +1288,9 @@
     B.tr.R = B.c.nT;
     B.filt = lds + 12 * B.c.nO + 8 * B.c.nT + PAD_FILT;
     B.filt_ok = false;
+#ifdef HFTLOB_STAMPS_CHUNK
+    B.a.n_resc = B.a.n_rec = B.b.n_resc = B.b.n_rec = 0;
+#endif
     B.a.scr = B.b.scr = B.tr.scr = lds + 12 * B.c.nO + 8 * B.c.nT + PAD_SCR;
     B.vs.init(B.c.nO);
     B.vt.init(B.c.nT);
@@ -1510,6 +1550,18 @@
     else return rt;
 }
 template <int BAKED> constexpr int baked_unroll() { return BAKED >= 0 ? HFTLOB_MAX_AGENTS : 1; }
+constexpr bool cfg_excl(const hftlob_env_cfg& c) {
+    bool ex = false;
+    for (int t = 0; t < c.n_types; ++t) ex |= c.types[t].kind == HFTLOB_AGENT_MM && c.types[t].exclude_extreme_spreads;
+    return ex;
+}
+template <int BAKED> constexpr bool baked_excl() {
+    if constexpr (BAKED == 0) return cfg_excl(hftlob_baked_cfg_0);
+    else if constexpr (BAKED == 1) return cfg_excl(hftlob_baked_cfg_1);
+    else if constexpr (BAKED == 2) return cfg_excl(hftlob_baked_cfg_2);
+    else if constexpr (BAKED == 3) return cfg_excl(hftlob_baked_cfg_3);
+    else return true;
+}
 
 template <int S, int BAKED = -1>
 DEV void env_reset_dev(const hftlob_env_cfg& c_rt, Key key, const i32* __restrict__ init_states, i32* __restrict__ rec,
@@ -2811,6 +2863,12 @@
     constexpr int UNR = baked_unroll<BAKED>();
     const bool emit = !QUIET && emit_rt;
     const bool vals = TALLY || emit;
+#ifdef HFTLOB_NO_LAZY
+    constexpr bool LZ_KERNEL = false;
+#else
+    constexpr bool LZ_KERNEL = NFIX > 0 && !RA && !baked_excl<BAKED>();
+#endif
+    constexpr bool LAZY = QUIET && LZ_KERNEL;
     STAMP(t_start);
 #ifdef HFTLOB_STAMPS
     const unsigned long long rt_start = __builtin_amdgcn_s_memrealtime();
@@ -2865,7 +2923,7 @@
             excl_any = ballot(any) != 0ull;
         }
     }
-    const bool store_best = NFIX == 0 || (!keep | excl_cfg);
+    const bool store_best = LAZY ? false : (NFIX == 0 || (!keep | excl_cfg));
     i32 dstart = wadd(start_index, wmul(D, step));
     dstart = imax_(0, imin_(dstart, c_rt.n_data_rows - D));
     const bool ftime = NFIX == 0 && c.ep_type == 1;
@@ -2879,7 +2937,7 @@
     if (resident) {
         relink_side(B.a, R, B.vs);
         relink_side(B.b, R, B.vs);
-        B.fl = fl_carry | F_STALE_A | F_STALE_B | STALE_ANY;
+        B.fl = (LZ_KERNEL ? fl_carry & ~F_LAZY : fl_carry) | F_STALE_A | F_STALE_B | STALE_ANY;
     } else {
         B.fl = commit_side<true>(B.a, fa, R, B.vs) | commit_side<false>(B.b, fb, R, B.vs) | F_STALE_A | F_STALE_B | STALE_ANY;
         B.fl |= slow_bit(B.fl);
@@ -3107,11 +3165,11 @@
     i32* carry = B.filt - PAD_FILT + PAD_CARRY;
     if (!RA && resident) {
         const i32 v = carry[l & 15];
-        B.a.best_p = rdl(v, 0); B.a.best_q = rdl(v, 1); B.a.xp = rdl(v, 2); B.a.top = rdl(v, 3);
+        B.a.best_p = rdl(v, 0); if (!LAZY) B.a.best_q = rdl(v, 1); B.a.xp = rdl(v, 2); B.a.top = rdl(v, 3);
         B.a.top_p = rdl(v, 4); B.a.top_ts = rdl(v, 5); B.a.top_tns = rdl(v, 6);
-        B.b.best_p = rdl(v, 7); B.b.best_q = rdl(v, 8); B.b.top = rdl(v, 9); B.b.top_p = rdl(v, 10);
+        B.b.best_p = rdl(v, 7); if (!LAZY) B.b.best_q = rdl(v, 8); B.b.top = rdl(v, 9); B.b.top_p = rdl(v, 10);
         B.b.top_ts = rdl(v, 11); B.b.top_tns = rdl(v, 12);
-        B.fl &= ~(F_STALE_A | F_STALE_B | STALE_ANY);
+        if (!(LZ_KERNEL && !LAZY && (fl_carry & F_LAZY))) B.fl &= ~(F_STALE_A | F_STALE_B | STALE_ANY);
     }
 #endif
 #ifdef HFTLOB_STAMPS_CHUNK
@@ -3153,7 +3211,7 @@
 #ifdef HFTLOB_STAMPS_CHUNK
         acc_dec += __builtin_amdgcn_s_memtime() - tc0;
 #endif
-        run_chunk<RC>(B, x, y, cnt, base, rpa, rqa, rpb, rqb CHUNK_ARGS);
+        run_chunk<RC, LAZY>(B, x, y, cnt, base, rpa, rqa, rpb, rqb CHUNK_ARGS);
 #ifdef HFTLOB_STAMPS_CHUNK
         const unsigned long long tc1 = __builtin_amdgcn_s_memtime();
 #endif
@@ -3167,7 +3225,13 @@
         const i32 cap = ffill(pa, prev_a), cbp = ffill(pb, prev_b);
         prev_a = rdl(cap, cnt - 1);
         prev_b = rdl(cbp, cnt - 1);
-        if ((row < M) & (store_best | (row == M - 1))) {
+        if (LAZY) {
+            if (row == M - 1) {
+                rec[c.off_best_asks + 2 * row] = cap;
+                rec[c.off_best_bids + 2 * row] = cbp;
+            }
+            (void)caq; (void)cbq;
+        } else if ((row < M) & (store_best | (row == M - 1))) {
             reinterpret_cast<int2*>(rec + c.off_best_asks)[row] = make_int2(cap, caq);
             reinterpret_cast<int2*>(rec + c.off_best_bids)[row] = make_int2(cbp, cbq);
         }
@@ -3192,9 +3256,11 @@
 #ifndef HFTLOB_NO_CARRY
     if (!RA && keep) {
         i32 v = B.a.best_p;
-        v = wlane(v, B.a.best_q, 1); v = wlane(v, B.a.xp, 2); v = wlane(v, B.a.top, 3); v = wlane(v, B.a.top_p, 4);
+        if (!LAZY) v = wlane(v, B.a.best_q, 1);
+        v = wlane(v, B.a.xp, 2); v = wlane(v, B.a.top, 3); v = wlane(v, B.a.top_p, 4);
         v = wlane(v, B.a.top_ts, 5); v = wlane(v, B.a.top_tns, 6); v = wlane(v, B.b.best_p, 7);
-        v = wlane(v, B.b.best_q, 8); v = wlane(v, B.b.top, 9); v = wlane(v, B.b.top_p, 10);
+        if (!LAZY) v = wlane(v, B.b.best_q, 8);
+        v = wlane(v, B.b.top, 9); v = wlane(v, B.b.top_p, 10);
         v = wlane(v, B.b.top_ts, 11); v = wlane(v, B.b.top_tns, 12);
         if (l < 13) carry[l] = v;
     }
@@ -3215,7 +3281,7 @@
     wv.vol_a = wv.vol_b = 0;
     if (emit) { wv.vol_a = side_volume(B.a, R, B.vs); wv.vol_b = side_volume(B.b, R, B.vs); }
     if (debug_out) write_debug(B, debug_out + (size_t)e * HFTLOB_DEBUG_WORDS(B.c.nT));
-    if (keep) fl_carry = B.fl;
+    if (keep) fl_carry = LAZY ? B.fl | F_LAZY : B.fl;
     if (!all & !keep) {
         store_side(B.a, rec + c.off_asks, R, B.vs);
         store_side(B.b, rec + c.off_bids, R, B.vs);
@@ -3360,7 +3426,7 @@
 #endif
 #ifdef HFTLOB_STAMPS_CHUNK
         info[9] = (i32)acc_dec; info[10] = (i32)acc_pre; info[11] = (i32)acc_loop; info[12] = (i32)acc_post;
-        info[13] = 0; info[14] = 0;
+        info[13] = (i32)(B.a.n_resc | (B.b.n_resc << 16)); info[14] = (i32)(B.a.n_rec | (B.b.n_rec << 16));
         (void)acc_act; (void)acc_cnl; (void)acc_flt; (void)acc_mmr; (void)acc_exr; (void)acc_obs;
 #else
         info[9] = (i32)acc_act; info[10] = (i32)acc_cnl; info[11] = (i32)acc_flt;
```

Result: faster. 104.4 million (median of 6 runs) (+2.0%).
